# qope/SIPP

Measured on NVIDIA B200. Metric: SIPP native prove throughput (pairings aggregated per second), higher is better.
Workload: dtype u32 limbs (254-bit modular integer)

## Files before the change

### include/sipp_b200.h

```cpp
#ifndef SIPP_B200_H
#define SIPP_B200_H
#include <stddef.h>
#include <stdint.h>

#ifdef __cplusplus
extern "C" {
#endif

typedef enum {
    SIPP_OK = 0,
    SIPP_ERR_CUDA = -1,
    SIPP_ERR_ARG = -2,
    SIPP_ERR_LENGTH = -3,
    SIPP_ERR_ZERO_CHALLENGE = -4,
    SIPP_ERR_SHORT_PROOF = -5,
    SIPP_ERR_ENCODING = -6,
    SIPP_ERR_VERIFY = -7,
    SIPP_ERR_COMM = -8
} sipp_status;

typedef struct sipp_ctx sipp_ctx;

int sipp_init(int device);
int sipp_shutdown(void);
const char *sipp_last_error(void);
int sipp_device_count(void);

#define SIPP_OPT_FE_NORMALISATION 1
#define SIPP_OPT_FQ12_ORDER 2
#define SIPP_OPT_PROFILE 3
#define SIPP_OPT_PIPELINE 4
#define SIPP_OPT_WIDE_LINES_MAX 5
#define SIPP_OPT_FE_ENGINE 6
#define SIPP_OPT_WIDE_FOLD_MAX 7
#define SIPP_OPT_WIDE_ACCUM_MAX 8
#define SIPP_OPT_BATCH_KPG_MAX 9
#define SIPP_OPT_FOLD_STRAUS 10
#define SIPP_OPT_BATCH_STREAMS 11
#define SIPP_OPT_BATCH_QLINES 12
#define SIPP_OPT_VALIDATE_POINTS 13
#define SIPP_OPT_MATRIX_TAIL 14
#define SIPP_OPT_MATRIX_BLOCK_N 15
#define SIPP_OPT_MATRIX_FIRST 17
#define SIPP_OPT_MATRIX_BLOCK_R 16
int sipp_set_option(int option, int value);
int sipp_get_option(int option);

int sipp_ctx_create(const uint8_t *A, const uint8_t *B, size_t n, sipp_ctx **out);
int sipp_ctx_create_from_device(const void *dA, const void *dB, size_t n, sipp_ctx **out);
int sipp_ctx_destroy(sipp_ctx *ctx);
size_t sipp_ctx_len(const sipp_ctx *ctx);
int sipp_ctx_inner_product(sipp_ctx *ctx, uint8_t out[384]);
int sipp_ctx_cross_products(sipp_ctx *ctx, uint8_t zl[384], uint8_t zr[384]);
int sipp_ctx_fold(sipp_ctx *ctx, const uint8_t x[32], const uint8_t x_inv[32]);
int sipp_ctx_set_stages(sipp_ctx *ctx, int on);
int sipp_ctx_read(sipp_ctx *ctx, uint8_t *A_out, uint8_t *B_out);

#define SIPP_PARTIAL_BYTES 384
int sipp_ctx_partial_products(sipp_ctx *ctx, int which, void *d_out, void *stream);
int sipp_combine_partials(const void *d_partials, int count, int nprod, uint8_t *out, void *stream);

#define SIPP_COMM_ID_BYTES 128
int sipp_comm_get_unique_id(uint8_t id[SIPP_COMM_ID_BYTES]);
int sipp_comm_init(const uint8_t id[SIPP_COMM_ID_BYTES], int rank, int world);
typedef int (*sipp_allgather_fn)(void *user, const void *send, void *recv, size_t bytes);
typedef int (*sipp_broadcast_fn)(void *user, void *buf, size_t bytes, int root);
int sipp_comm_init_host(int rank, int world, sipp_allgather_fn allgather, sipp_broadcast_fn broadcast, void *user);
int sipp_comm_destroy(void);
int sipp_comm_rank(void);
int sipp_comm_world(void);
int sipp_comm_nccl_version(void);
int sipp_prove_native_sharded(const uint8_t *A_local, const uint8_t *B_local, size_t n, const uint8_t *A_full, const uint8_t *B_full,
                              uint8_t *proof);
int sipp_prove_native_sharded_device(const void *dA_local, const void *dB_local, size_t n, const uint8_t *A_full, const uint8_t *B_full,
                                     uint8_t *proof);
#define SIPP_SHARD_XS_BYTES 72
typedef struct sipp_shard_backend {
    void *user;
    int rank, world;
    size_t (*local_len)(void *user);
    int (*products)(void *user, int which);
    int (*combine)(void *user, int nprod, uint8_t *out);
    int (*broadcast)(void *user, uint8_t *xs);
    int (*fold)(void *user, const uint8_t *x, const uint8_t *x_inv);
    int (*collapse)(void *user);
} sipp_shard_backend;
int sipp_prove_native_sharded_backend(const sipp_shard_backend *backend, size_t n, const uint8_t *A_full, const uint8_t *B_full,
                                      uint8_t *proof);

int sipp_pairing(const uint8_t a[64], const uint8_t b[128], uint8_t out[384]);
int sipp_inner_product(const uint8_t *A, const uint8_t *B, size_t n, uint8_t out[384]);
int sipp_fr_inverse(const uint8_t x[32], uint8_t out[32]);
int sipp_gt_fold(const uint8_t zl[384], const uint8_t z[384], const uint8_t zr[384], const uint8_t x[32],
                 const uint8_t x_inv[32], uint8_t out[384]);

typedef struct { uint64_t state[4]; } sipp_transcript;
void sipp_transcript_new(sipp_transcript *t);
void sipp_transcript_append(sipp_transcript *t, const uint64_t *msg, size_t n);
void sipp_transcript_append_fq12(sipp_transcript *t, const uint8_t f[384]);
void sipp_transcript_append_g1(sipp_transcript *t, const uint8_t a[64]);
void sipp_transcript_append_g2(sipp_transcript *t, const uint8_t b[128]);
void sipp_transcript_get_challenge(const sipp_transcript *t, uint8_t x[32]);
void sipp_transcript_append_pairs(sipp_transcript *t, const uint8_t *A, const uint8_t *B, size_t n);
void sipp_poseidon_permute(uint64_t state[12]);
void sipp_poseidon_permute_portable(uint64_t state[12]);
int sipp_poseidon_backend(void);
double sipp_poseidon_ns_per_permutation(long count);

int sipp_prove_native(const uint8_t *A, size_t a_len, const uint8_t *B, size_t b_len, uint8_t *proof);
size_t sipp_proof_len(size_t n);
int sipp_ctx_prove(sipp_ctx *ctx, const uint8_t *A, const uint8_t *B, uint8_t *proof);
int sipp_verify_native(const uint8_t *A, size_t a_len, const uint8_t *B, size_t b_len, const uint8_t *proof, size_t proof_len,
                       uint8_t *final_A, uint8_t *final_B, uint8_t *final_Z);

size_t sipp_statement_u32_len(size_t n);
int sipp_statement_to_u32(const uint8_t *A, const uint8_t *B, size_t n, const uint8_t Z[384], const uint8_t final_A[64],
                          const uint8_t final_B[128], const uint8_t final_Z[384], uint32_t *out, size_t out_len);
int sipp_statement_from_u32(size_t n, const uint32_t *in, size_t in_len, uint8_t *A, uint8_t *B, uint8_t Z[384], uint8_t final_A[64],
                            uint8_t final_B[128], uint8_t final_Z[384]);

int sipp_prove_native_batch(const uint8_t *A, const uint8_t *B, size_t n, size_t count, uint8_t *proofs);
int sipp_verify_native_batch(const uint8_t *A, const uint8_t *B, size_t n, size_t count, const uint8_t *proofs, size_t proof_len,
                             int *results, uint8_t *final_A, uint8_t *final_B, uint8_t *final_Z);
int sipp_prove_native_batch_device(const void *dA, const void *dB, size_t n, size_t count, void *d_proofs);

int sipp_g1_generator_mul_batch(const uint8_t *scalars, size_t count, uint8_t *out);
int sipp_g1_generator_mul_batch_device(const void *d_scalars, size_t count, void *d_out);
int sipp_g2_mul_batch(const uint8_t *points, size_t point_count, const uint8_t *scalars, size_t count, uint8_t *out);
int sipp_g2_mul_batch_device(const void *d_points, size_t point_count, const void *d_scalars, size_t count, void *d_out);
int sipp_g2_sum(const uint8_t *points, size_t count, uint8_t out[128]);
int sipp_g2_sum_device(const void *d_points, size_t count, void *d_out);
int sipp_g1_neg_generator(uint8_t out[64]);

int sipp_seeded_inputs_device(uint64_t seed, size_t n, void *dA, void *dB);
int sipp_seeded_inputs(uint64_t seed, size_t n, uint8_t *A, uint8_t *B);

typedef struct {
    uint64_t launches;
    uint64_t miller_pairs;
    uint64_t miller_launches;
    double miller_ms;
    double reduce_fe_ms;
    double fold_ms;
    uint64_t fold_points;
    double transcript_ms;
    double other_ms;
} sipp_stats;
int sipp_get_stats(sipp_stats *out);
int sipp_reset_stats(void);

int sipp_test_fq_op(int op, const uint8_t *a, const uint8_t *b, uint8_t *out, size_t count);
int sipp_test_fq12_op(int op, const uint8_t *a, const uint8_t *b, uint8_t *out, size_t count);
int sipp_test_fold_plan(const uint8_t x[32], const uint8_t x_inv[32], uint32_t *out_words, size_t out_cap);
int sipp_test_poseidon_device(uint64_t *states, size_t count);
int sipp_test_transcript_round_device(uint64_t *states, const uint8_t *fq12s, int nf, size_t count, uint8_t *x_out, uint32_t *plans_out);
int sipp_test_fr_inverse_binary(const uint8_t x[32], uint8_t out[32]);
int sipp_microbench(int which, int iters, double *ops_per_s, double *ms);
long sipp_test_stage_blocks(int which, size_t n);
long sipp_test_poseidon_chain(uint64_t seed, long count);
int sipp_test_poseidon_scalar(int which, const uint64_t *in, uint64_t *out);
const void *sipp_test_poseidon_tables(void);

#ifdef __cplusplus
}
#endif
#endif
```

### sipp_b200/_lib.py

```python
import ctypes
import os

_HERE = os.path.dirname(os.path.abspath(__file__))
LIB_PATH = os.environ.get("SIPP_LIB") or os.path.join(_HERE, "libsipp_b200.so")

OK, ERR_CUDA, ERR_ARG, ERR_LENGTH, ERR_ZERO_CHALLENGE, ERR_SHORT_PROOF, ERR_ENCODING, ERR_VERIFY, ERR_COMM = 0, -1, -2, -3, -4, -5, -6, -7, -8
OPT_FE_NORMALISATION, OPT_FQ12_ORDER, OPT_PROFILE, OPT_PIPELINE, OPT_WIDE_LINES_MAX, OPT_FE_ENGINE, OPT_WIDE_FOLD_MAX, OPT_WIDE_ACCUM_MAX = 1, 2, 3, 4, 5, 6, 7, 8
OPT_BATCH_KPG_MAX, OPT_FOLD_STRAUS, OPT_BATCH_STREAMS, OPT_BATCH_QLINES, OPT_VALIDATE_POINTS, OPT_MATRIX_TAIL, OPT_MATRIX_BLOCK_N, OPT_MATRIX_BLOCK_R, OPT_MATRIX_FIRST = 9, 10, 11, 12, 13, 14, 15, 16, 17


class SippError(RuntimeError):
    def __init__(self, code, msg):
        super().__init__("libsipp_b200 error %d: %s" % (code, msg))
        self.code = code


class Stats(ctypes.Structure):
    _fields_ = [("launches", ctypes.c_uint64), ("miller_pairs", ctypes.c_uint64), ("miller_launches", ctypes.c_uint64),
                ("miller_ms", ctypes.c_double), ("reduce_fe_ms", ctypes.c_double), ("fold_ms", ctypes.c_double),
                ("fold_points", ctypes.c_uint64), ("transcript_ms", ctypes.c_double), ("other_ms", ctypes.c_double)]


class TranscriptState(ctypes.Structure):
    _fields_ = [("state", ctypes.c_uint64 * 4)]


ALLGATHER_FN = ctypes.CFUNCTYPE(ctypes.c_int, ctypes.c_void_p, ctypes.c_void_p, ctypes.c_void_p, ctypes.c_size_t)
BROADCAST_FN = ctypes.CFUNCTYPE(ctypes.c_int, ctypes.c_void_p, ctypes.c_void_p, ctypes.c_size_t, ctypes.c_int)
SHARD_XS_BYTES = 72


class ShardBackend(ctypes.Structure):
    LEN_FN = ctypes.CFUNCTYPE(ctypes.c_size_t, ctypes.c_void_p)
    PRODUCTS_FN = ctypes.CFUNCTYPE(ctypes.c_int, ctypes.c_void_p, ctypes.c_int)
    COMBINE_FN = ctypes.CFUNCTYPE(ctypes.c_int, ctypes.c_void_p, ctypes.c_int, ctypes.c_void_p)
    BROADCAST_FN = ctypes.CFUNCTYPE(ctypes.c_int, ctypes.c_void_p, ctypes.c_void_p)
    FOLD_FN = ctypes.CFUNCTYPE(ctypes.c_int, ctypes.c_void_p, ctypes.c_void_p, ctypes.c_void_p)
    COLLAPSE_FN = ctypes.CFUNCTYPE(ctypes.c_int, ctypes.c_void_p)
    _fields_ = [("user", ctypes.c_void_p), ("rank", ctypes.c_int), ("world", ctypes.c_int), ("local_len", LEN_FN), ("products", PRODUCTS_FN),
                ("combine", COMBINE_FN), ("broadcast", BROADCAST_FN), ("fold", FOLD_FN), ("collapse", COLLAPSE_FN)]


_lib = None


def load():
    global _lib
    if _lib is not None:
        return _lib
    if not os.path.exists(LIB_PATH):
        raise SippError(ERR_CUDA, "%s not built: run `python -c 'import __graft_entry__ as g; g.build()'` "
                                  "(there is no CPU fallback)" % LIB_PATH)
    lib = ctypes.CDLL(LIB_PATH)
    vp, sz, u8p, i = ctypes.c_void_p, ctypes.c_size_t, ctypes.c_char_p, ctypes.c_int
    lib.sipp_last_error.restype = ctypes.c_char_p
    lib.sipp_ctx_create.argtypes = [u8p, u8p, sz, ctypes.POINTER(vp)]
    lib.sipp_poseidon_ns_per_permutation.argtypes = [ctypes.c_long]
    lib.sipp_poseidon_ns_per_permutation.restype = ctypes.c_double
    lib.sipp_ctx_create_from_device.argtypes = [vp, vp, sz, ctypes.POINTER(vp)]
    lib.sipp_ctx_destroy.argtypes = [vp]
    lib.sipp_ctx_len.argtypes = [vp]
    lib.sipp_ctx_len.restype = sz
    lib.sipp_ctx_inner_product.argtypes = [vp, u8p]
    lib.sipp_ctx_cross_products.argtypes = [vp, u8p, u8p]
    lib.sipp_ctx_fold.argtypes = [vp, u8p, u8p]
    lib.sipp_ctx_read.argtypes = [vp, u8p, u8p]
    lib.sipp_ctx_set_stages.argtypes = [vp, ctypes.c_int]
    lib.sipp_ctx_partial_products.argtypes = [vp, i, vp, vp]
    lib.sipp_combine_partials.argtypes = [vp, i, i, u8p, vp]
    lib.sipp_pairing.argtypes = [u8p, u8p, u8p]
    lib.sipp_inner_product.argtypes = [u8p, u8p, sz, u8p]
    lib.sipp_fr_inverse.argtypes = [u8p, u8p]
    lib.sipp_gt_fold.argtypes = [u8p, u8p, u8p, u8p, u8p, u8p]
    lib.sipp_transcript_new.argtypes = [ctypes.POINTER(TranscriptState)]
    lib.sipp_transcript_new.restype = None
    lib.sipp_transcript_append.argtypes = [ctypes.POINTER(TranscriptState), ctypes.POINTER(ctypes.c_uint64), sz]
    lib.sipp_transcript_append.restype = None
    for name in ("sipp_transcript_append_fq12", "sipp_transcript_append_g1", "sipp_transcript_append_g2"):
        getattr(lib, name).argtypes = [ctypes.POINTER(TranscriptState), u8p]
        getattr(lib, name).restype = None
    lib.sipp_transcript_get_challenge.argtypes = [ctypes.POINTER(TranscriptState), u8p]
    lib.sipp_transcript_get_challenge.restype = None
    lib.sipp_transcript_append_pairs.argtypes = [ctypes.POINTER(TranscriptState), u8p, u8p, sz]
    lib.sipp_transcript_append_pairs.restype = None
    lib.sipp_poseidon_permute.argtypes = [ctypes.POINTER(ctypes.c_uint64)]
    lib.sipp_poseidon_permute.restype = None
    lib.sipp_prove_native.argtypes = [u8p, sz, u8p, sz, u8p]
    lib.sipp_proof_len.argtypes = [sz]
    lib.sipp_proof_len.restype = sz
    lib.sipp_ctx_prove.argtypes = [vp, u8p, u8p, u8p]
    lib.sipp_verify_native.argtypes = [u8p, sz, u8p, sz, u8p, sz, u8p, u8p, u8p]
    lib.sipp_seeded_inputs_device.argtypes = [ctypes.c_uint64, sz, vp, vp]
    lib.sipp_seeded_inputs.argtypes = [ctypes.c_uint64, sz, u8p, u8p]
    lib.sipp_get_stats.argtypes = [ctypes.POINTER(Stats)]
    lib.sipp_test_fq_op.argtypes = [i, u8p, u8p, u8p, sz]
    lib.sipp_test_fq12_op.argtypes = [i, u8p, u8p, u8p, sz]
    lib.sipp_prove_native_batch.argtypes = [u8p, u8p, sz, sz, u8p]
    lib.sipp_prove_native_batch_device.argtypes = [vp, vp, sz, sz, vp]
    lib.sipp_verify_native_batch.argtypes = [u8p, u8p, sz, sz, u8p, sz, ctypes.POINTER(ctypes.c_int), u8p, u8p, u8p]
    lib.sipp_test_poseidon_device.argtypes = [ctypes.POINTER(ctypes.c_uint64), sz]
    lib.sipp_test_transcript_round_device.argtypes = [ctypes.POINTER(ctypes.c_uint64), u8p, i, sz, u8p, ctypes.POINTER(ctypes.c_uint32)]
    lib.sipp_test_fold_plan.argtypes = [u8p, u8p, ctypes.POINTER(ctypes.c_uint32), sz]
    u32p = ctypes.POINTER(ctypes.c_uint32)
    lib.sipp_statement_u32_len.argtypes = [sz]
    lib.sipp_statement_u32_len.restype = sz
    lib.sipp_statement_to_u32.argtypes = [u8p, u8p, sz, u8p, u8p, u8p, u8p, u32p, sz]
    lib.sipp_statement_from_u32.argtypes = [sz, u32p, sz, u8p, u8p, u8p, u8p, u8p, u8p]
    lib.sipp_g1_generator_mul_batch.argtypes = [u8p, sz, u8p]
    lib.sipp_g1_generator_mul_batch_device.argtypes = [vp, sz, vp]
    lib.sipp_g2_mul_batch.argtypes = [u8p, sz, u8p, sz, u8p]
    lib.sipp_g2_mul_batch_device.argtypes = [vp, sz, vp, sz, vp]
    lib.sipp_g2_sum.argtypes = [u8p, sz, u8p]
    lib.sipp_g2_sum_device.argtypes = [vp, sz, vp]
    lib.sipp_g1_neg_generator.argtypes = [u8p]
    lib.sipp_comm_get_unique_id.argtypes = [u8p]
    lib.sipp_comm_init.argtypes = [u8p, i, i]
    lib.sipp_comm_init_host.argtypes = [i, i, ALLGATHER_FN, BROADCAST_FN, vp]
    lib.sipp_prove_native_sharded.argtypes = [u8p, u8p, sz, u8p, u8p, u8p]
    lib.sipp_prove_native_sharded_device.argtypes = [vp, vp, sz, u8p, u8p, u8p]
    lib.sipp_prove_native_sharded_backend.argtypes = [ctypes.POINTER(ShardBackend), sz, u8p, u8p, u8p]
    lib.sipp_microbench.argtypes = [i, i, ctypes.POINTER(ctypes.c_double), ctypes.POINTER(ctypes.c_double)]
    _lib = lib
    return lib


def check(rc):
    if rc != OK:
        raise SippError(rc, load().sipp_last_error().decode("utf-8", "replace"))
    return rc


def require_gpu(device=0):
    check(load().sipp_init(device))


_gpu_ready = False


def require_gpu_once():
    global _gpu_ready
    if not _gpu_ready:
        dev = int(os.environ.get("LOCAL_RANK", "0")) if "SIPP_DEVICE" not in os.environ else int(os.environ["SIPP_DEVICE"])
        require_gpu(dev)
        _gpu_ready = True
```

### sipp_b200/csrc/fold_plan.h

```cpp
#pragma once
#include <stdint.h>

namespace sipp {

#define SIPP_FOLD_MASK_WORDS 5

struct FoldSubScalar {
    uint64_t mag[3];
    int neg;
};
struct FoldComp {
    uint32_t plus[SIPP_FOLD_MASK_WORDS];
    uint32_t minus[SIPP_FOLD_MASK_WORDS];
    int neg;
};
struct FoldPlan {
    FoldComp g1[2];
    FoldComp g2[4];
    int g1_bits, g2_bits;
};

struct GtPlan {
    FoldComp c[8];
    int bits;
};

int fold_decompose_g1(const uint64_t k[4], FoldSubScalar out[2]);
int fold_decompose_g2(const uint64_t k[4], FoldSubScalar out[4]);
int fold_plan_build(const uint8_t x[32], const uint8_t x_inv[32], FoldPlan* plan);
int gt_plan_build(const uint8_t x[32], const uint8_t x_inv[32], GtPlan* plan);

}
```

### sipp_b200/csrc/glv.cc

```cpp
#include <string.h>

#include "glv_consts.h"
#include "glv_core.h"

namespace sipp {

static const glv::Tables HOST_TABLES = {&SIPP_GLV_G1_BASIS[0][0][0], &SIPP_GLV_G1_RECIP[0][0], SIPP_GLV_G1_RECIP_SIGN,
                                        &SIPP_GLS_G2_BASIS[0][0][0], &SIPP_GLS_G2_RECIP[0][0], SIPP_GLS_G2_RECIP_SIGN};

int fold_decompose_g2(const uint64_t k[4], FoldSubScalar out[4]) {
    return glv::decompose<4>(k, HOST_TABLES.g2_basis, HOST_TABLES.g2_recip, HOST_TABLES.g2_sign, out);
}
int fold_decompose_g1(const uint64_t k[4], FoldSubScalar out[2]) {
    return glv::decompose<2>(k, HOST_TABLES.g1_basis, HOST_TABLES.g1_recip, HOST_TABLES.g1_sign, out);
}

int fold_plan_build(const uint8_t x[32], const uint8_t x_inv[32], FoldPlan* plan) {
    uint64_t kx[4], ki[4];
    memcpy(kx, x, 32);
    memcpy(ki, x_inv, 32);
    memset(plan, 0, sizeof *plan);
    return glv::plan_build(kx, ki, HOST_TABLES, plan);
}

int gt_plan_build(const uint8_t x[32], const uint8_t x_inv[32], GtPlan* plan) {
    memset(plan, 0, sizeof *plan);
    for (int which = 0; which < 2; which++) {
        uint64_t k[4];
        memcpy(k, which ? x_inv : x, 32);
        FoldSubScalar s[4];
        if (fold_decompose_g2(k, s)) return -1;
        for (int j = 0; j < 4; j++) {
            FoldComp& c = plan->c[4 * which + j];
            const int len = glv::naf(s[j].mag, c.plus, c.minus);
            c.neg = s[j].neg;
            if (len > plan->bits) plan->bits = len;
        }
    }
    return plan->bits > 32 * SIPP_FOLD_MASK_WORDS ? -1 : 0;
}

}

extern "C" int sipp_test_fr_inverse_binary(const uint8_t x[32], uint8_t out[32]) {
    uint64_t v[4], o[4] = {0, 0, 0, 0};
    memcpy(v, x, 32);
    int rc = sipp::glv::fr_inverse_binary(v, o);
    memcpy(out, o, 32);
    return rc;
}
```

### sipp_b200/csrc/host_state.h

```cpp
#pragma once
#include <cuda_runtime.h>
#include <stddef.h>
#include <stdint.h>

#include <atomic>
#include <thread>

#include "../../include/sipp_b200.h"
#include "launch.h"

namespace sipp_host {
void pool_free(void* p);
struct MatTail {
    uint32_t* E[2] = {nullptr, nullptr};
    int cur = 0;
    size_t n = 0;
    size_t m = 1;
    bool fold_points = false;
    int folds = 0;
    void reset() {
        pool_free(E[0]);
        pool_free(E[1]);
        E[0] = E[1] = nullptr;
        n = 0;
        m = 1;
        fold_points = false;
    }
    ~MatTail() { reset(); }
};
}

struct sipp_ctx {
    uint32_t* dA = nullptr;
    uint32_t* dB = nullptr;
    size_t n = 0, cap = 0;
    bool stages = false;
    bool stale = false;
    bool pending_validation = false;
    cudaEvent_t validated = nullptr;
    sipp_host::MatTail mt;
};

namespace sipp_host {

extern int g_device;
extern int g_sm_count;
extern cudaStream_t g_stream;
#define SIPP_FIRST_STAGE_LOG2_LOOPS 18
size_t mat_first_budget(size_t n);
extern int g_opt_pipeline, g_opt_fe_norm, g_opt_fq12_order, g_opt_profile, g_opt_fold_straus, g_opt_batch_kpg_max, g_opt_batch_streams, g_opt_batch_qlines, g_opt_wide_max, g_opt_wide_fold_max, g_opt_fe_engine, g_opt_validate, g_opt_matrix_n, g_opt_matrix_first, g_opt_matrix_block_n, g_opt_matrix_block_r;
extern sipp_stats g_stats;

int fail(int code, const char* what);
int cuda_fail(cudaError_t e, const char* what);
int ensure_init();
bool is_pow2(size_t n);

void batch_release_streams();
int ctx_alloc(size_t n, sipp_ctx** out);
inline bool fq_bytes_canonical(const uint8_t* b, size_t n_fq) {
    static const uint64_t PM[4] = {0x3c208c16d87cfd47ull, 0x97816a916871ca8dull, 0xb85045b68181585dull, 0x30644e72e131a029ull};
    for (size_t i = 0; i < n_fq; i++) {
        uint64_t w[4];
        __builtin_memcpy(w, b + 32 * i, 32);
        bool less = false;
        for (int k = 3; k >= 0; k--) {
            if (w[k] != PM[k]) { less = w[k] < PM[k]; break; }
        }
        if (!less) return false;
    }
    return true;
}
cudaError_t pool_alloc(void** out, size_t bytes);
int lines_reserve(size_t bytes);
uint32_t* lines_buffer();
cudaError_t order_after(cudaStream_t later, cudaStream_t earlier);

struct AbsorbJob {
    sipp_transcript tr;
    std::thread th;
    std::atomic<bool> cancel{false};
    void start(const uint8_t* A, const uint8_t* B, size_t n) {
        sipp_transcript_new(&tr);
        th = std::thread([this, A, B, n]() {
            const size_t chunk = 512;
            for (size_t i = 0; i < n && !cancel.load(std::memory_order_relaxed); i += chunk)
                sipp_transcript_append_pairs(&tr, A + 64 * i, B + 128 * i, n - i < chunk ? n - i : chunk);
        });
    }
    double join();
    ~AbsorbJob() {
        cancel.store(true);
        if (th.joinable()) th.join();
    }
};

size_t mat_stage_first(size_t n);
int mat_diag_product(MatTail& mt, uint8_t* z);
size_t mat_stage(size_t n);
int mat_build(sipp_ctx* c, MatTail& mt, size_t nr);
int mat_build_ex(sipp_ctx* c, MatTail& mt, size_t nr, uint32_t* raw_out);
int mat_adopt(MatTail& mt, const uint32_t* gathered, int ranks, size_t nr);
int mat_products(MatTail& mt, uint8_t* zl, uint8_t* zr);
int mat_fold(sipp_ctx* c, MatTail& mt, const uint8_t x[32], const uint8_t xinv[32]);

int prove_core(sipp_ctx* c, AbsorbJob& job, uint8_t* proof);

int span_begin(int kind, cudaStream_t s);
void span_end(int idx, cudaStream_t s);
struct Span {
    int idx;
    cudaStream_t stream;
    Span(int kind, cudaStream_t s) : idx(span_begin(kind, s)), stream(s) {}
    ~Span() { span_end(idx, stream); }
};

}

#define CK(call)                                                    \
    do {                                                            \
        cudaError_t e_ = (call);                                    \
        if (e_ != cudaSuccess) return sipp_host::cuda_fail(e_, #call); \
    } while (0)
```

### sipp_b200/csrc/k_fold.cu

```cuda
#define SIPP_CURVE_FQ2_CALLS 1
#define SIPP_FQ_CALLS 1
#include "coop.cuh"
#include "device_common.cuh"
#include "fold_plan.h"
#include "fq2h.cuh"

namespace sipp {

#define SIPP_FOLD_THREADS 128

template <class F>
__device__ __forceinline__ void store_jac(uint32_t* dst, const Jac<F>& p);
template <>
__device__ __forceinline__ void store_jac<Fq2>(uint32_t* dst, const Jac<Fq2>& p) {
    store_fq2_words(dst, p.x); store_fq2_words(dst + 16, p.y); store_fq2_words(dst + 32, p.z);
}
__device__ __forceinline__ Jac<Fq2> load_jac2(const uint32_t* src) {
    Jac<Fq2> p;
    p.x = load_fq2_words(src); p.y = load_fq2_words(src + 16); p.z = load_fq2_words(src + 32);
    return p;
}
__device__ __forceinline__ void store_fq_words(uint32_t* p, const Fq& v) {
    uint4* q = reinterpret_cast<uint4*>(p);
    q[0] = make_uint4(v.l[0], v.l[1], v.l[2], v.l[3]);
    q[1] = make_uint4(v.l[4], v.l[5], v.l[6], v.l[7]);
}
__device__ __forceinline__ Fq load_fq_words(const uint32_t* p) {
    const uint4* q = reinterpret_cast<const uint4*>(p);
    uint4 a = q[0], b = q[1];
    return Fq{{a.x, a.y, a.z, a.w, b.x, b.y, b.z, b.w}};
}
template <>
__device__ __forceinline__ void store_jac<Fq>(uint32_t* dst, const Jac<Fq>& p) {
    store_fq_words(dst, p.x); store_fq_words(dst + 8, p.y); store_fq_words(dst + 16, p.z);
}
__device__ __forceinline__ Jac<Fq> load_jac1(const uint32_t* src) {
    Jac<Fq> p;
    p.x = load_fq_words(src); p.y = load_fq_words(src + 8); p.z = load_fq_words(src + 16);
    return p;
}

__device__ __forceinline__ void store_jac_h(uint32_t* dst, const Jac<Fq2H>& p) {
    const int o = h_odd() ? 8 : 0;
    store_fq_words(dst + o, p.x.v); store_fq_words(dst + 16 + o, p.y.v); store_fq_words(dst + 32 + o, p.z.v);
}
__device__ __forceinline__ Jac<Fq2H> load_jac_h(const uint32_t* src) {
    const int o = h_odd() ? 8 : 0;
    Jac<Fq2H> p;
    p.x.v = load_fq_words(src + o); p.y.v = load_fq_words(src + 16 + o); p.z.v = load_fq_words(src + 32 + o);
    return p;
}
__device__ __forceinline__ Affine<Fq2H> split_g2(const G2A& q) { return Affine<Fq2H>{h_split(q.x), h_split(q.y)}; }

__device__ __forceinline__ void pair_mul(const Fq& a_even, const Fq& b_even, const Fq& a_odd, const Fq& b_odd, Fq& r_even, Fq& r_odd) {
    const bool odd = h_odd();
    const Fq mine = fq_mul_call(h_select(odd, a_odd, a_even), h_select(odd, b_odd, b_even));
    const Fq other = h_partner(mine);
    r_even = h_select(odd, other, mine);
    r_odd = h_select(odd, mine, other);
}
__device__ __noinline__ Jac<Fq> jac_dbl_pair(const Jac<Fq>& p) {
    Fq A, B, C, S, Fv, YZ, M, unused;
    pair_mul(p.x, p.x, p.y, p.y, A, B);
    const Fq xb = fq_add(p.x, B);
    pair_mul(B, B, xb, xb, C, S);
    const Fq D = fq_dbl(fq_sub(fq_sub(S, A), C));
    const Fq E = fq_add(fq_dbl(A), A);
    pair_mul(E, E, p.y, p.z, Fv, YZ);
    Jac<Fq> r;
    r.x = fq_sub(Fv, fq_dbl(D));
    const Fq dx = fq_sub(D, r.x);
    pair_mul(E, dx, E, dx, M, unused);
    r.y = fq_sub(M, fq_dbl(fq_dbl(fq_dbl(C))));
    r.z = fq_dbl(YZ);
    return r;
}
__device__ __noinline__ Jac<Fq> jac_add_affine_pair(const Jac<Fq>& p, const G1A& q) {
    if (affine_is_identity(q)) return p;
    if (fq_is_zero(p.z)) return Jac<Fq>{q.x, q.y, fq_one()};
    Fq zz, yz, u2, s2, hh, zh, hhh, v, r2, yh, M, unused;
    pair_mul(p.z, p.z, q.y, p.z, zz, yz);
    pair_mul(q.x, zz, yz, zz, u2, s2);
    const Fq h = fq_sub(u2, p.x), rr = fq_sub(s2, p.y);
    if (fq_is_zero(h)) {
        if (fq_is_zero(rr)) return jac_dbl_pair(p);
        return jac_identity<Fq>();
    }
    pair_mul(h, h, p.z, h, hh, zh);
    pair_mul(hh, h, p.x, hh, hhh, v);
    pair_mul(rr, rr, p.y, hhh, r2, yh);
    Jac<Fq> r;
    r.x = fq_sub(fq_sub(fq_sub(r2, hhh), v), v);
    const Fq vx = fq_sub(v, r.x);
    pair_mul(rr, vx, rr, vx, M, unused);
    r.y = fq_sub(M, yh);
    r.z = zh;
    return r;
}
__device__ __forceinline__ Jac<Fq> jac_scalar_mul_naf_pair(const G1A& q, const uint32_t* plus, const uint32_t* minus, int bits) {
    Jac<Fq> acc = jac_identity<Fq>();
    for (int i = bits - 1; i >= 0; i--) {
        acc = jac_dbl_pair(acc);
        const uint32_t m = 1u << (i & 31);
        const bool dp = (plus[i >> 5] & m) != 0, dm = (minus[i >> 5] & m) != 0;
        if (dp || dm) {
            G1A t = q;
            if (dm) t.y = fq_neg(q.y);
            acc = jac_add_affine_pair(acc, t);
        }
    }
    return acc;
}

template <class F>
__device__ __forceinline__ Jac<F> fold_component(const Affine<F>& p2, const FoldComp& c, int j, int bits) {
    Affine<F> q = endo_apply(p2, j);
    if (c.neg) q.y = f_neg(q.y);
    return jac_scalar_mul_naf(q, c.plus, c.minus, bits);
}

__global__ void __launch_bounds__(SIPP_FOLD_THREADS) k_fold_split(uint32_t* __restrict__ A, uint32_t* __restrict__ B, size_t h, FoldPlan plan_arg,
                                                                 unsigned g2_blocks) {
    __shared__ FoldPlan plan;
    __shared__ __align__(16) uint32_t xch[3 * 32 * 48];
    for (int i = threadIdx.x; i < (int)(sizeof(FoldPlan) / 4); i += blockDim.x) ((uint32_t*)&plan)[i] = ((const uint32_t*)&plan_arg)[i];
    __syncthreads();
    const int warp = threadIdx.x >> 5, lane = threadIdx.x & 31;
    if (blockIdx.x < g2_blocks) {
        const int el = lane >> 1;
        size_t i = (size_t)blockIdx.x * 16 + el;
        const bool valid = i < h;
        if (!valid) i = h - 1;
        G2A q = endo_apply(load_g2(B, i + h), warp);
        if (plan.g2[warp].neg) q.y = f_neg(q.y);
        Jac<Fq2H> acc = jac_scalar_mul_naf(split_g2(q), plan.g2[warp].plus, plan.g2[warp].minus, plan.g2_bits);
        if (warp > 0) store_jac_h(xch + ((warp - 1) * 16 + el) * 48, acc);
        __syncthreads();
        if (warp == 0) {
#pragma unroll 1
            for (int j = 0; j < 3; j++) acc = jac_add(acc, load_jac_h(xch + (j * 16 + el) * 48));
            const Affine<Fq2H> r = jac_to_affine(jac_add_affine(acc, split_g2(load_g2(B, i))));
            if (valid) {
                const int o = h_odd() ? 8 : 0;
                store_fq_words(B + 32 * i + o, r.x.v);
                store_fq_words(B + 32 * i + 16 + o, r.y.v);
            }
        }
    } else {
        const int comp = warp & 1, half = warp >> 1, el = lane >> 1;
        size_t i = (size_t)(blockIdx.x - g2_blocks) * 32 + half * 16 + el;
        const bool valid = i < h;
        if (!valid) i = h - 1;
        G1A q = endo_apply(load_g1(A, i + h), comp);
        if (plan.g1[comp].neg) q.y = fq_neg(q.y);
        Jac<Fq> acc = jac_scalar_mul_naf_pair(q, plan.g1[comp].plus, plan.g1[comp].minus, plan.g1_bits);
        if (comp == 1 && !h_odd()) store_jac(xch + (half * 16 + el) * 24, acc);
        __syncthreads();
        if (comp == 0 && !h_odd()) {
            acc = jac_add(acc, load_jac1(xch + (half * 16 + el) * 24));
            G1A r = jac_to_affine(jac_add_affine(acc, load_g1(A, i)));
            if (valid) store_g1(A, i, r);
        }
    }
}


__global__ void __launch_bounds__(SIPP_FOLD_THREADS) k_fold_batch(uint32_t* __restrict__ A, uint32_t* __restrict__ B, size_t h, size_t stride, size_t count,
                                                                 const FoldPlan* __restrict__ plans, unsigned g2_blocks) {
    __shared__ __align__(16) uint32_t xch[3 * 16 * 48];
    const int warp = threadIdx.x >> 5, lane = threadIdx.x & 31, el = lane >> 1;
    const size_t total = count * h;
    if (blockIdx.x < g2_blocks) {
        size_t e = (size_t)blockIdx.x * 16 + el;
        const bool valid = e < total;
        if (!valid) e = total - 1;
        const size_t inst = e / h, i = inst * stride + e % h;
        const FoldPlan* pl = plans + inst;
        G2A q = endo_apply(load_g2(B, i + h), warp);
        if (pl->g2[warp].neg) q.y = f_neg(q.y);
        Jac<Fq2H> acc = jac_scalar_mul_naf(split_g2(q), pl->g2[warp].plus, pl->g2[warp].minus, pl->g2_bits);
        if (warp > 0) store_jac_h(xch + ((warp - 1) * 16 + el) * 48, acc);
        __syncthreads();
        if (warp == 0) {
#pragma unroll 1
            for (int j = 0; j < 3; j++) acc = jac_add(acc, load_jac_h(xch + (j * 16 + el) * 48));
            const Affine<Fq2H> r = jac_to_affine(jac_add_affine(acc, split_g2(load_g2(B, i))));
            if (valid) {
                const int o = h_odd() ? 8 : 0;
                store_fq_words(B + 32 * i + o, r.x.v);
                store_fq_words(B + 32 * i + 16 + o, r.y.v);
            }
        }
    } else {
        const int comp = warp & 1, half = warp >> 1;
        size_t e = (size_t)(blockIdx.x - g2_blocks) * 32 + half * 16 + el;
        const bool valid = e < total;
        if (!valid) e = total - 1;
        const size_t inst = e / h, i = inst * stride + e % h;
        const FoldPlan* pl = plans + inst;
        G1A q = endo_apply(load_g1(A, i + h), comp);
        if (pl->g1[comp].neg) q.y = fq_neg(q.y);
        Jac<Fq> acc = jac_scalar_mul_naf_pair(q, pl->g1[comp].plus, pl->g1[comp].minus, pl->g1_bits);
        if (comp == 1 && !h_odd()) store_jac(xch + (half * 16 + el) * 24, acc);
        __syncthreads();
        if (comp == 0 && !h_odd()) {
            acc = jac_add(acc, load_jac1(xch + (half * 16 + el) * 24));
            G1A r = jac_to_affine(jac_add_affine(acc, load_g1(A, i)));
            if (valid) store_g1(A, i, r);
        }
    }
}

#define SIPP_STRAUS_THREADS 64

__global__ void __launch_bounds__(SIPP_STRAUS_THREADS) k_fold_straus(uint32_t* __restrict__ A, uint32_t* __restrict__ B, size_t h, size_t stride, size_t count,
                                                                   const FoldPlan* __restrict__ plans, unsigned g2_blocks) {
    const size_t total = count * h;
    const bool is_g2 = blockIdx.x < g2_blocks;
    size_t e = (size_t)(is_g2 ? blockIdx.x : blockIdx.x - g2_blocks) * SIPP_STRAUS_THREADS + threadIdx.x;
    if (e >= total) return;
    const size_t inst = e / h, i = inst * stride + e % h;
    const FoldPlan* pl = plans + inst;
    if (is_g2) {
        G2A tbl[4];
        const G2A p2 = load_g2(B, i + h);
#pragma unroll 1
        for (int c = 0; c < 4; c++) {
            tbl[c] = endo_apply(p2, c);
            if (pl->g2[c].neg) tbl[c].y = f_neg(tbl[c].y);
        }
        Jac<Fq2> acc = straus_naf<Fq2, 4>(tbl, pl->g2, pl->g2_bits);
        store_g2(B, i, jac_to_affine(jac_add_affine(acc, load_g2(B, i))));
    } else {
        G1A tbl[2];
        const G1A p2 = load_g1(A, i + h);
#pragma unroll 1
        for (int c = 0; c < 2; c++) {
            tbl[c] = endo_apply(p2, c);
            if (pl->g1[c].neg) tbl[c].y = f_neg(tbl[c].y);
        }
        Jac<Fq> acc = straus_naf<Fq, 2>(tbl, pl->g1, pl->g1_bits);
        store_g1(A, i, jac_to_affine(jac_add_affine(acc, load_g1(A, i))));
    }
}

__device__ __forceinline__ Jac<Fq2> psi_jac(const Jac<Fq2>& p, int j) {
    Jac<Fq2> r;
    r.x = f_mul((j & 1) ? fq2_conj(p.x) : p.x, frob_gamma(j, 2));
    r.y = f_mul((j & 1) ? fq2_conj(p.y) : p.y, frob_gamma(j, 3));
    r.z = (j & 1) ? fq2_conj(p.z) : p.z;
    return r;
}
__device__ bool jac_equal(const Jac<Fq2>& p, const Jac<Fq2>& q) {
    const bool pz = f_is_zero(p.z), qz = f_is_zero(q.z);
    if (pz || qz) return pz && qz;
    const Fq2 z1 = f_sqr(p.z), z2 = f_sqr(q.z);
    if (!fq2_eq(f_mul(p.x, z2), f_mul(q.x, z1))) return false;
    return fq2_eq(f_mul(p.y, f_mul(z2, q.z)), f_mul(q.y, f_mul(z1, p.z)));
}
__global__ void __launch_bounds__(64) k_validate_points(const uint32_t* __restrict__ dA, const uint32_t* __restrict__ dB, size_t n, int* __restrict__ flags) {
    const size_t t = (size_t)blockIdx.x * blockDim.x + threadIdx.x;
    if (t >= 2 * n) return;
    if (t < n) {
        const G1A p{load_fq_words(dA + 16 * t), load_fq_words(dA + 16 * t + 8)};
        if (affine_is_identity(p)) return;
        const Fq three = fq_to_mont(Fq{{3, 0, 0, 0, 0, 0, 0, 0}});
        if (!f_is_zero(f_sub(f_sqr(p.y), f_add(f_mul(f_sqr(p.x), p.x), three)))) atomicOr(flags, 2);
        return;
    }
    const size_t i = t - n;
    const G2A q{load_fq2_words(dB + 32 * i), load_fq2_words(dB + 32 * i + 16)};
    if (affine_is_identity(q)) return;
    if (!fq2_eq(f_sqr(q.y), f_add(f_mul(f_sqr(q.x), q.x), fq2_b_twist()))) { atomicOr(flags, 2); return; }
    const unsigned long long xb = SIPP_BN_X;
    const uint32_t k[8] = {(uint32_t)xb, (uint32_t)(xb >> 32), 0, 0, 0, 0, 0, 0};
    const Jac<Fq2> xq = jac_scalar_mul(q, k);
    Jac<Fq2> lhs = jac_add_affine(xq, q);
    lhs = jac_add(lhs, psi_jac(xq, 1));
    lhs = jac_add(lhs, psi_jac(xq, 2));
    const Jac<Fq2> rhs = psi_jac(jac_dbl(xq), 3);
    if (!jac_equal(lhs, rhs)) atomicOr(flags, 4);
}
int launch_validate_points(const uint32_t* dA, const uint32_t* dB, size_t n, int* flags, cudaStream_t s) {
    k_validate_points<<<(unsigned)((2 * n + 63) / 64), 64, 0, s>>>(dA, dB, n, flags);
    return (int)cudaGetLastError();
}

int launch_fold(uint32_t* A, uint32_t* B, size_t h, const FoldPlan& plan, cudaStream_t s) {
    unsigned g2_blocks = (unsigned)((h + 15) / 16), g1_blocks = (unsigned)((h + 31) / 32);
    k_fold_split<<<g2_blocks + g1_blocks, SIPP_FOLD_THREADS, 0, s>>>(A, B, h, plan, g2_blocks);
    return (int)cudaGetLastError();
}
int launch_fold_batch(uint32_t* A, uint32_t* B, size_t h, size_t stride, size_t count, const FoldPlan* plans, cudaStream_t s) {
    size_t total = count * h;
    unsigned g2_blocks = (unsigned)((total + 15) / 16), g1_blocks = (unsigned)((total + 31) / 32);
    k_fold_batch<<<g2_blocks + g1_blocks, SIPP_FOLD_THREADS, 0, s>>>(A, B, h, stride, count, plans, g2_blocks);
    return (int)cudaGetLastError();
}
int launch_fold_straus(uint32_t* A, uint32_t* B, size_t h, size_t stride, size_t count, const FoldPlan* plans, cudaStream_t s) {
    size_t total = count * h;
    unsigned blocks = (unsigned)((total + SIPP_STRAUS_THREADS - 1) / SIPP_STRAUS_THREADS);
    k_fold_straus<<<2 * blocks, SIPP_STRAUS_THREADS, 0, s>>>(A, B, h, stride, count, plans, blocks);
    return (int)cudaGetLastError();
}

}
```

### sipp_b200/csrc/k_wide.cu

```cuda
#include "engine.cuh"
#include "device_common.cuh"

namespace sipp {

#define SIPP_WIDE_THREADS 128
#define SIPP_WIDE_GROUPS (SIPP_WIDE_THREADS / SIPP_LP_LANES)
#define SIPP_LINE_WORDS 80

static __device__ const LpIns d_lp_code[SIPP_LP_LEVELS * SIPP_LP_LANES] = SIPP_LP_CODE_INIT;
static __constant__ unsigned char c_lp_types[SIPP_LP_LEVELS] = SIPP_LP_TYPES_INIT;

struct DevMachine {
    uint32_t* slots;
    uint32_t* out;
    int lane;
    bool store, ident;
    __device__ __forceinline__ void run(int first, int n) {
#pragma unroll 1
        for (int L = first; L < first + n; L++) {
            const uint4 w = __ldg(reinterpret_cast<const uint4*>(d_lp_code) + L * SIPP_LP_LANES + lane);
            const LpIns ins{w.x, w.y, w.z, w.w};
            const Fq r = lp_eval(c_lp_types[L], ins, slots);
            __syncwarp();
            lp_store(slots, lp_dst(ins), r);
            __syncwarp();
        }
    }
    __device__ __forceinline__ void emit(int step) {
        if (lane < 10 && store) {
            Fq v = lp_load(slots, SIPP_LP_SLOT_OUT0 + lane);
            if (ident) v = (lane == 0) ? fq_one() : fq_zero();
            uint4* o = reinterpret_cast<uint4*>(out + (size_t)step * SIPP_LINE_WORDS + lane * 8);
            o[0] = make_uint4(v.l[0], v.l[1], v.l[2], v.l[3]);
            o[1] = make_uint4(v.l[4], v.l[5], v.l[6], v.l[7]);
        }
    }
};

__global__ void __launch_bounds__(SIPP_WIDE_THREADS) k_lines_wide(const uint32_t* __restrict__ A, const uint32_t* __restrict__ B, MillerJob job, int nprod,
                                                                 size_t c0, size_t mc, uint32_t* __restrict__ lines) {
    __shared__ __align__(16) uint32_t smem[SIPP_WIDE_GROUPS * SIPP_LP_SLOTS * 8];
    __shared__ int ident_flag[SIPP_WIDE_GROUPS];
    const int group = threadIdx.x / SIPP_LP_LANES, lane = threadIdx.x % SIPP_LP_LANES;
    const size_t total = mc * (size_t)nprod;
    size_t t = (size_t)blockIdx.x * SIPP_WIDE_GROUPS + group;
    const bool valid = t < total;
    if (!valid) t = total - 1;
    const int prod = (int)(t / mc);
    const size_t j = c0 + (t - (size_t)prod * mc);
    uint32_t* slots = smem + group * (SIPP_LP_SLOTS * 8);
    if (lane == 0) {
        const G1A p = load_g1(A, job.a_off[prod] + j);
        const G2A q = load_g2(B, job.b_off[prod] + j);
        ident_flag[group] = (affine_is_identity(p) || affine_is_identity(q)) ? 1 : 0;
        lp_fill_fixed(slots, p.x, p.y, q.x, q.y);
    }
    __syncwarp();
    DevMachine mach;
    mach.slots = slots;
    mach.out = lines + t * (size_t)(SIPP_LINES_PER_PAIR * SIPP_LINE_WORDS);
    mach.lane = lane;
    mach.store = valid;
    mach.ident = ident_flag[group] != 0;
    lp_miller(mach);
}

__global__ void __launch_bounds__(SIPP_WIDE_THREADS) k_lines_wide_batch(const uint32_t* __restrict__ A, const uint32_t* __restrict__ B, BatchJob job, size_t p0,
                                                                       size_t np, uint32_t* __restrict__ lines) {
    __shared__ __align__(16) uint32_t smem[SIPP_WIDE_GROUPS * SIPP_LP_SLOTS * 8];
    __shared__ int ident_flag[SIPP_WIDE_GROUPS];
    const int group = threadIdx.x / SIPP_LP_LANES, lane = threadIdx.x % SIPP_LP_LANES;
    const size_t total = np * job.h;
    size_t t = (size_t)blockIdx.x * SIPP_WIDE_GROUPS + group;
    const bool valid = t < total;
    if (!valid) t = total - 1;
    const size_t P = p0 + t / job.h, i = t % job.h;
    const size_t inst = P / (size_t)job.nprod;
    const int y = (int)(P % (size_t)job.nprod);
    const size_t base = inst * job.stride + i;
    uint32_t* slots = smem + group * (SIPP_LP_SLOTS * 8);
    if (lane == 0) {
        const G1A p = load_g1(A, base + job.a_off[y]);
        const G2A q = load_g2(B, base + job.b_off[y]);
        ident_flag[group] = (affine_is_identity(p) || affine_is_identity(q)) ? 1 : 0;
        lp_fill_fixed(slots, p.x, p.y, q.x, q.y);
    }
    __syncwarp();
    DevMachine mach;
    mach.slots = slots;
    mach.out = lines + t * (size_t)(SIPP_LINES_PER_PAIR * SIPP_LINE_WORDS);
    mach.lane = lane;
    mach.store = valid;
    mach.ident = ident_flag[group] != 0;
    lp_miller(mach);
}

int launch_lines_wide_batch(const uint32_t* A, const uint32_t* B, const BatchJob& job, size_t p0, size_t np, uint32_t* lines, cudaStream_t s) {
    const size_t groups = np * job.h;
    k_lines_wide_batch<<<(unsigned)((groups + SIPP_WIDE_GROUPS - 1) / SIPP_WIDE_GROUPS), SIPP_WIDE_THREADS, 0, s>>>(A, B, job, p0, np, lines);
    return (int)cudaGetLastError();
}

int launch_lines_wide(const uint32_t* A, const uint32_t* B, const MillerJob& job, int nprod, size_t c0, size_t mc, uint32_t* lines, cudaStream_t s) {
    const size_t groups = mc * (size_t)nprod;
    k_lines_wide<<<(unsigned)((groups + SIPP_WIDE_GROUPS - 1) / SIPP_WIDE_GROUPS), SIPP_WIDE_THREADS, 0, s>>>(A, B, job, nprod, c0, mc, lines);
    return (int)cudaGetLastError();
}

}

namespace sipp {

__device__ __forceinline__ void store_words(uint32_t* dst, const Fq& v) {
#pragma unroll
    for (int i = 0; i < 8; i++) dst[i] = v.l[i];
}
__device__ __forceinline__ Fq load_words(const uint32_t* src) {
    Fq v;
#pragma unroll
    for (int i = 0; i < 8; i++) v.l[i] = src[i];
    return v;
}

__global__ void __launch_bounds__(SIPP_WIDE_THREADS) k_fold_wide(uint32_t* __restrict__ A, uint32_t* __restrict__ B, size_t h, FoldPlan plan_arg, unsigned g2_blocks) {
    __shared__ __align__(16) uint32_t smem[SIPP_WIDE_GROUPS * SIPP_LP_SLOTS * 8];
    __shared__ FoldPlan plan;
    __shared__ __align__(16) uint32_t xch[SIPP_WIDE_GROUPS * 48];
    for (int i = threadIdx.x; i < (int)(sizeof(FoldPlan) / 4); i += blockDim.x) ((uint32_t*)&plan)[i] = ((const uint32_t*)&plan_arg)[i];
    __syncthreads();
    const int warp = threadIdx.x >> 5, group = threadIdx.x / SIPP_LP_LANES, lane = threadIdx.x % SIPP_LP_LANES, gi = group & 1;
    uint32_t* slots = smem + group * (SIPP_LP_SLOTS * 8);
    DevMachine mach;
    mach.slots = slots; mach.out = nullptr; mach.lane = lane; mach.store = false; mach.ident = false;
    if (blockIdx.x < g2_blocks) {
        const int comp = warp;
        size_t e = (size_t)blockIdx.x * 2 + gi;
        const bool valid = e < h;
        if (!valid) e = h - 1;
        const FoldDigits d = fold_digits(plan.g2[comp], plan.g2_bits);
        bool ident = false;
        if (lane == 0) {
            G2A q = load_g2(B, e + h);
            ident = affine_is_identity(q);
            q = endo_apply(q, comp);
            if ((plan.g2[comp].neg != 0) != d.flip) q.y = fq2_neg(q.y);
            lp_fill_fixed(slots, fq_zero(), fq_zero(), q.x, q.y);
        }
        __syncwarp();
        if (d.top >= 0) {
            mach.run(SIPP_LP_SETUP_FIRST, SIPP_LP_SETUP_LEVELS);
            lp_scalar_mul(mach, true, d.plus, d.minus, d.top);
        }
        if (lane == 0) {
            Jac<Fq2> r = jac_identity<Fq2>();
            if (!ident && d.top >= 0) {
                const Fq2 X{lp_load(slots, SIPP_LP_SLOT_X0), lp_load(slots, SIPP_LP_SLOT_X1)}, Y{lp_load(slots, SIPP_LP_SLOT_Y0), lp_load(slots, SIPP_LP_SLOT_Y1)};
                const Fq2 Z = fq2_mul_xi(Fq2{lp_load(slots, SIPP_LP_SLOT_ZH0), lp_load(slots, SIPP_LP_SLOT_ZH1)});
                r.x = fq2_mul(X, Z);
                r.y = fq2_mul(Y, fq2_sqr(Z));
                r.z = Z;
            }
            uint32_t* o = xch + group * 48;
            store_words(o, r.x.c0); store_words(o + 8, r.x.c1); store_words(o + 16, r.y.c0); store_words(o + 24, r.y.c1);
            store_words(o + 32, r.z.c0); store_words(o + 40, r.z.c1);
        }
        __syncthreads();
        if (warp == 0 && lane == 0) {
            Jac<Fq2> acc;
            for (int j = 0; j < 4; j++) {
                const uint32_t* o = xch + ((j * 2 + gi) * 48);
                Jac<Fq2> t;
                t.x = Fq2{load_words(o), load_words(o + 8)}; t.y = Fq2{load_words(o + 16), load_words(o + 24)}; t.z = Fq2{load_words(o + 32), load_words(o + 40)};
                acc = j ? jac_add(acc, t) : t;
            }
            const G2A r = jac_to_affine(jac_add_affine(acc, load_g2(B, e)));
            if (valid) store_g2(B, e, r);
        }
    } else {
        const int comp = warp & 1, pair = warp >> 1;
        size_t e = (size_t)(blockIdx.x - g2_blocks) * 4 + pair * 2 + gi;
        const bool valid = e < h;
        if (!valid) e = h - 1;
        const FoldDigits d = fold_digits(plan.g1[comp], plan.g1_bits);
        bool ident = false;
        if (lane == 0) {
            G1A q = load_g1(A, e + h);
            ident = affine_is_identity(q);
            q = endo_apply(q, comp);
            if ((plan.g1[comp].neg != 0) != d.flip) q.y = fq_neg(q.y);
            lp_store(slots, SIPP_LP_SLOT_ZERO, fq_zero());
            lp_store(slots, SIPP_LP_SLOT_QX0, q.x); lp_store(slots, SIPP_LP_SLOT_QY0, q.y);
            lp_store(slots, SIPP_LP_SLOT_X1, q.x); lp_store(slots, SIPP_LP_SLOT_Y1, q.y); lp_store(slots, SIPP_LP_SLOT_Z1, fq_one());
        }
        __syncwarp();
        if (d.top >= 0) lp_scalar_mul(mach, false, d.plus, d.minus, d.top);
        if (lane == 0) {
            Jac<Fq> r = jac_identity<Fq>();
            if (!ident && d.top >= 0) {
                const Fq X = lp_load(slots, SIPP_LP_SLOT_X1), Y = lp_load(slots, SIPP_LP_SLOT_Y1), Z = lp_load(slots, SIPP_LP_SLOT_Z1);
                r.x = fq_mul(X, Z);
                r.y = fq_mul(Y, fq_sqr(Z));
                r.z = Z;
            }
            uint32_t* o = xch + group * 48;
            store_words(o, r.x); store_words(o + 8, r.y); store_words(o + 16, r.z);
        }
        __syncthreads();
        if (comp == 0 && lane == 0) {
            Jac<Fq> acc, t;
            const uint32_t* o0 = xch + group * 48;
            const uint32_t* o1 = xch + (group + 2) * 48;
            acc.x = load_words(o0); acc.y = load_words(o0 + 8); acc.z = load_words(o0 + 16);
            t.x = load_words(o1); t.y = load_words(o1 + 8); t.z = load_words(o1 + 16);
            acc = jac_add(acc, t);
            const G1A r = jac_to_affine(jac_add_affine(acc, load_g1(A, e)));
            if (valid) store_g1(A, e, r);
        }
    }
}

__global__ void __launch_bounds__(SIPP_WIDE_THREADS) k_fold_wide_batch(uint32_t* __restrict__ A, uint32_t* __restrict__ B, size_t h, size_t stride, size_t count,
                                                                      const FoldPlan* __restrict__ plans, unsigned g2_blocks) {
    __shared__ __align__(16) uint32_t smem[SIPP_WIDE_GROUPS * SIPP_LP_SLOTS * 8];
    __shared__ __align__(16) uint32_t xch[SIPP_WIDE_GROUPS * 48];
    const size_t total = count * h;
    const int epw = h >= 2 ? 2 : 1;
    const int warp = threadIdx.x >> 5, group = threadIdx.x / SIPP_LP_LANES, lane = threadIdx.x % SIPP_LP_LANES, gi = group & 1;
    uint32_t* slots = smem + group * (SIPP_LP_SLOTS * 8);
    DevMachine mach;
    mach.slots = slots; mach.out = nullptr; mach.lane = lane; mach.store = false; mach.ident = false;
    if (blockIdx.x < g2_blocks) {
        const int comp = warp;
        size_t E = (size_t)blockIdx.x * epw + (gi % epw);
        const bool valid = E < total && gi < epw;
        if (E >= total) E = total - 1;
        const size_t inst = E / h, e = inst * stride + E % h;
        const FoldPlan& plan = plans[inst];
        const FoldDigits d = fold_digits(plan.g2[comp], plan.g2_bits);
        bool ident = false;
        if (lane == 0) {
            G2A q = load_g2(B, e + h);
            ident = affine_is_identity(q);
            q = endo_apply(q, comp);
            if ((plan.g2[comp].neg != 0) != d.flip) q.y = fq2_neg(q.y);
            lp_fill_fixed(slots, fq_zero(), fq_zero(), q.x, q.y);
        }
        __syncwarp();
        if (d.top >= 0) {
            mach.run(SIPP_LP_SETUP_FIRST, SIPP_LP_SETUP_LEVELS);
            lp_scalar_mul(mach, true, d.plus, d.minus, d.top);
        }
        if (lane == 0) {
            Jac<Fq2> r = jac_identity<Fq2>();
            if (!ident && d.top >= 0) {
                const Fq2 X{lp_load(slots, SIPP_LP_SLOT_X0), lp_load(slots, SIPP_LP_SLOT_X1)}, Y{lp_load(slots, SIPP_LP_SLOT_Y0), lp_load(slots, SIPP_LP_SLOT_Y1)};
                const Fq2 Z = fq2_mul_xi(Fq2{lp_load(slots, SIPP_LP_SLOT_ZH0), lp_load(slots, SIPP_LP_SLOT_ZH1)});
                r.x = fq2_mul(X, Z);
                r.y = fq2_mul(Y, fq2_sqr(Z));
                r.z = Z;
            }
            uint32_t* o = xch + group * 48;
            store_words(o, r.x.c0); store_words(o + 8, r.x.c1); store_words(o + 16, r.y.c0); store_words(o + 24, r.y.c1);
            store_words(o + 32, r.z.c0); store_words(o + 40, r.z.c1);
        }
        __syncthreads();
        if (warp == 0 && lane == 0) {
            Jac<Fq2> acc;
            for (int j = 0; j < 4; j++) {
                const uint32_t* o = xch + ((j * 2 + gi) * 48);
                Jac<Fq2> t;
                t.x = Fq2{load_words(o), load_words(o + 8)}; t.y = Fq2{load_words(o + 16), load_words(o + 24)}; t.z = Fq2{load_words(o + 32), load_words(o + 40)};
                acc = j ? jac_add(acc, t) : t;
            }
            const G2A r = jac_to_affine(jac_add_affine(acc, load_g2(B, e)));
            if (valid) store_g2(B, e, r);
        }
    } else {
        const int comp = warp & 1, pair = warp >> 1;
        size_t E = (size_t)(blockIdx.x - g2_blocks) * (2 * epw) + pair * epw + (gi % epw);
        const bool valid = E < total && gi < epw;
        if (E >= total) E = total - 1;
        const size_t inst = E / h, e = inst * stride + E % h;
        const FoldPlan& plan = plans[inst];
        const FoldDigits d = fold_digits(plan.g1[comp], plan.g1_bits);
        bool ident = false;
        if (lane == 0) {
            G1A q = load_g1(A, e + h);
            ident = affine_is_identity(q);
            q = endo_apply(q, comp);
            if ((plan.g1[comp].neg != 0) != d.flip) q.y = fq_neg(q.y);
            lp_store(slots, SIPP_LP_SLOT_ZERO, fq_zero());
            lp_store(slots, SIPP_LP_SLOT_QX0, q.x); lp_store(slots, SIPP_LP_SLOT_QY0, q.y);
            lp_store(slots, SIPP_LP_SLOT_X1, q.x); lp_store(slots, SIPP_LP_SLOT_Y1, q.y); lp_store(slots, SIPP_LP_SLOT_Z1, fq_one());
        }
        __syncwarp();
        if (d.top >= 0) lp_scalar_mul(mach, false, d.plus, d.minus, d.top);
        if (lane == 0) {
            Jac<Fq> r = jac_identity<Fq>();
            if (!ident && d.top >= 0) {
                const Fq X = lp_load(slots, SIPP_LP_SLOT_X1), Y = lp_load(slots, SIPP_LP_SLOT_Y1), Z = lp_load(slots, SIPP_LP_SLOT_Z1);
                r.x = fq_mul(X, Z);
                r.y = fq_mul(Y, fq_sqr(Z));
                r.z = Z;
            }
            uint32_t* o = xch + group * 48;
            store_words(o, r.x); store_words(o + 8, r.y); store_words(o + 16, r.z);
        }
        __syncthreads();
        if (comp == 0 && lane == 0) {
            Jac<Fq> acc, t;
            const uint32_t* o0 = xch + group * 48;
            const uint32_t* o1 = xch + (group + 2) * 48;
            acc.x = load_words(o0); acc.y = load_words(o0 + 8); acc.z = load_words(o0 + 16);
            t.x = load_words(o1); t.y = load_words(o1 + 8); t.z = load_words(o1 + 16);
            acc = jac_add(acc, t);
            const G1A r = jac_to_affine(jac_add_affine(acc, load_g1(A, e)));
            if (valid) store_g1(A, e, r);
        }
    }
}


int launch_fold_wide_batch(uint32_t* A, uint32_t* B, size_t h, size_t stride, size_t count, const FoldPlan* plans, cudaStream_t s) {
    const size_t total = count * h, epw = h >= 2 ? 2 : 1;
    const unsigned g2_blocks = (unsigned)((total + epw - 1) / epw), g1_blocks = (unsigned)((total + 2 * epw - 1) / (2 * epw));
    k_fold_wide_batch<<<g2_blocks + g1_blocks, SIPP_WIDE_THREADS, 0, s>>>(A, B, h, stride, count, plans, g2_blocks);
    return (int)cudaGetLastError();
}
int launch_fold_wide(uint32_t* A, uint32_t* B, size_t h, const FoldPlan& plan, cudaStream_t s) {
    const unsigned g2_blocks = (unsigned)((h + 1) / 2), g1_blocks = (unsigned)((h + 3) / 4);
    k_fold_wide<<<g2_blocks + g1_blocks, SIPP_WIDE_THREADS, 0, s>>>(A, B, h, plan, g2_blocks);
    return (int)cudaGetLastError();
}

}
```

### sipp_b200/csrc/launch.h

```cpp
#pragma once
#include <cuda_runtime.h>
#include <stddef.h>
#include <stdint.h>

#include "fold_plan.h"

namespace sipp {

struct MillerJob {
    size_t a_off[2];
    size_t b_off[2];
    size_t m;
};
struct BatchJob {
    size_t stride;
    size_t a_off[2];
    size_t b_off[2];
    size_t h;
    int nprod;
};
struct Scalar256 {
    uint32_t w[8];
};

#define SIPP_MILLER_BLOCK 64

int launch_codec_decode(const uint32_t* in, uint32_t* out, size_t n_fq, int* flags, cudaStream_t s);
int launch_codec_encode(const uint32_t* in, uint32_t* out, size_t n_fq, cudaStream_t s);
int launch_miller_block(const uint32_t* A, const uint32_t* B, const MillerJob& job, int nprod, uint32_t* partials, cudaStream_t s);
int launch_reduce_fe(const uint32_t* partials, int count, int nprod, uint32_t* out, int final_exp, int ark_norm, cudaStream_t s);
int launch_gt_fold(const uint32_t* in, const Scalar256& x, const Scalar256& xinv, uint32_t* out, cudaStream_t s);
int launch_gt_fold_eng(const uint32_t* in, const Scalar256& x, const Scalar256& xinv, uint32_t* out, cudaStream_t s);
int launch_gt_fold_rounds(const uint32_t* elems, const uint32_t* scalars, int rounds, uint32_t* partials, cudaStream_t s);
int launch_fold(uint32_t* A, uint32_t* B, size_t h, const FoldPlan& plan, cudaStream_t s);
int launch_fold_wide(uint32_t* A, uint32_t* B, size_t h, const FoldPlan& plan, cudaStream_t s);
int launch_validate_points(const uint32_t* dA, const uint32_t* dB, size_t n, int* flags, cudaStream_t s);
int launch_test_fq_op(int op, const uint32_t* a, const uint32_t* b, uint32_t* out, size_t count, cudaStream_t s);
int launch_test_fq12_op(int op, const uint32_t* a, const uint32_t* b, uint32_t* out, size_t count, cudaStream_t s);
int launch_microbench(int which, int blocks, int threads, void* out, int iters, uint32_t seed, double* ops_per_thread, cudaStream_t s);

int launch_lines(const uint32_t* A, const uint32_t* B, const MillerJob& job, int nprod, size_t c0, size_t mc, uint32_t* lines, cudaStream_t s);
int launch_lines_wide(const uint32_t* A, const uint32_t* B, const MillerJob& job, int nprod, size_t c0, size_t mc, uint32_t* lines, cudaStream_t s);
int accum_blocks(size_t m_chunk, int kpg);
int launch_accum(const uint32_t* lines, size_t m_chunk, int nprod, int kpg, uint32_t* partials, int block_offset, cudaStream_t s);
int launch_reduce_fe_coop(const uint32_t* partials, int count, int nprod, uint32_t* out, int final_exp, int ark_norm, cudaStream_t s);
int launch_reduce_fe_eng(const uint32_t* partials, int count, int nprod, uint32_t* out, int final_exp, int ark_norm, cudaStream_t s);
int accum_eng_blocks(size_t m_chunk, int kpg);
int launch_accum_eng(const uint32_t* lines, size_t m_chunk, int nprod, int kpg, uint32_t* partials, int block_offset, cudaStream_t s);
int launch_accum_eng_each(const uint32_t* lines, size_t m, uint32_t* out, cudaStream_t s);
int launch_test_coop_op(int op, const uint32_t* a, const uint32_t* b, uint32_t* out, size_t count, cudaStream_t s);
size_t lines_bytes_per_pair();

int launch_mat_gather(const uint32_t* A, const uint32_t* B, size_t nr, size_t m, uint32_t* Aexp, uint32_t* Bexp, cudaStream_t s);
int launch_mat_fe(const uint32_t* miller, size_t count, uint32_t* E, int ark_norm, cudaStream_t s);
int launch_mat_diag(const uint32_t* E, size_t n, int main_diagonal, uint32_t* partials, cudaStream_t s);
int launch_mat_fold(const uint32_t* E, size_t n, uint32_t* Eout, const GtPlan& plan, cudaStream_t s);

int launch_lines_batch(const uint32_t* A, const uint32_t* B, const BatchJob& job, size_t p0, size_t np, uint32_t* lines, cudaStream_t s);
int launch_accum_batch(const uint32_t* lines, size_t pairs, int kpg, uint32_t* partials, size_t group_offset, cudaStream_t s);
int launch_fe_batch(const uint32_t* partials, size_t nproducts, int gpp, int nprod, uint32_t* out, size_t out_stride, int slot0, int slot1, int ark_norm,
                    cudaStream_t s);
int launch_lines_wide_batch(const uint32_t* A, const uint32_t* B, const BatchJob& job, size_t p0, size_t np, uint32_t* lines, cudaStream_t s);
int launch_qlines_batch(const uint32_t* B, size_t npoints, uint32_t* qlines, cudaStream_t s);
int launch_eval_lines_batch(const uint32_t* A, const uint32_t* B, const BatchJob& job, size_t p0, size_t np, const uint32_t* qlines, uint32_t* lines,
                            cudaStream_t s);
size_t qlines_bytes_per_point();
int launch_eval_lines_mat(const uint32_t* A, const uint32_t* B, size_t nr, size_t m, const uint32_t* qlines, uint32_t* lines, cudaStream_t s);
int launch_fe_batch_eng(const uint32_t* partials, size_t nproducts, int gpp, int nprod, uint32_t* out, size_t out_stride, int slot0, int slot1, int ark_norm,
                        cudaStream_t s);
int launch_fold_batch(uint32_t* A, uint32_t* B, size_t h, size_t stride, size_t count, const FoldPlan* plans, cudaStream_t s);
int launch_fold_wide_batch(uint32_t* A, uint32_t* B, size_t h, size_t stride, size_t count, const FoldPlan* plans, cudaStream_t s);
int launch_fold_straus(uint32_t* A, uint32_t* B, size_t h, size_t stride, size_t count, const FoldPlan* plans, cudaStream_t s);
int launch_tr_absorb_pairs(const uint32_t* bytesA, const uint32_t* bytesB, size_t n, size_t count, uint64_t* states, cudaStream_t s);
int launch_tr_round(uint64_t* states, const uint32_t* proofs, size_t np, int slot_z, int slot_l, int slot_r, int order, size_t count, FoldPlan* plans,
                    uint64_t* challenges, int* flags, cudaStream_t s);
int launch_test_poseidon(uint64_t* states, size_t count, cudaStream_t s);
int launch_gt_fold_batch(const uint32_t* proofs, size_t stride, int slot_l, int slot_r, const uint64_t* challenges, uint32_t* z, size_t count,
                         cudaStream_t s);

size_t window_table_bytes(int group);
int launch_window_table(int group, const uint32_t* base, uint32_t* table, cudaStream_t s);
int launch_fixed_base_mul(int group, const uint32_t* table, const uint32_t* scalars, size_t count, uint32_t* out, cudaStream_t s);
int launch_g2_mul_var(const uint32_t* points, const uint32_t* scalars, size_t count, uint32_t* out, cudaStream_t s);
int g2_sum_blocks(size_t count, int sm_count);
int launch_g2_sum(const uint32_t* points, size_t count, uint32_t* partials, int blocks, uint32_t* out, cudaStream_t s);
int launch_seeded_scalars(uint64_t seed, size_t n, uint32_t* sa, uint32_t* sb, cudaStream_t s);
int launch_generators(uint32_t* gens, cudaStream_t s);

}
```

### sipp_b200/csrc/sipp_b200.cu

```cuda
#include <cuda_runtime.h>
#include <stdio.h>
#include <string.h>

#include <chrono>
#include <string>
#include <thread>
#include <vector>

#include "glv_core.h"
#include "host_state.h"

using namespace sipp;

namespace sipp_host {

thread_local std::string g_err;
int g_device = -1;
cudaStream_t g_stream = nullptr;
int g_opt_fe_norm = 0, g_opt_fq12_order = 0, g_opt_profile = 0, g_opt_pipeline = 1;
int g_opt_fe_engine = 1;
int g_opt_wide_fold_max = 256;
int g_opt_wide_accum_max = 1536;
int g_opt_wide_max = 8192;
int g_sm_count = 148;
int g_opt_fold_straus = 1;
int g_opt_batch_streams = 0;
int g_opt_batch_qlines = 1;
int g_opt_batch_kpg_max = 32;
int g_opt_matrix_n = 32;
int g_opt_matrix_first = 1;
int g_opt_matrix_block_n = 256, g_opt_matrix_block_r = 8;
int g_opt_validate = 1;

struct TimedSpan {
    cudaEvent_t a, b;
    int kind;
};
std::vector<TimedSpan> g_spans;
sipp_stats g_stats;

int fail(int code, const char* what) {
    g_err = what;
    return code;
}
int cuda_fail(cudaError_t e, const char* what) {
    g_err = std::string(what) + ": " + cudaGetErrorString(e);
    return SIPP_ERR_CUDA;
}
int ensure_init() {
    if (g_device >= 0) return SIPP_OK;
    return sipp_init(0);
}

int span_begin(int kind, cudaStream_t s) {
    if (!g_opt_profile) return -1;
    TimedSpan t;
    t.kind = kind;
    cudaEventCreate(&t.a);
    cudaEventCreate(&t.b);
    cudaEventRecord(t.a, s);
    g_spans.push_back(t);
    return (int)g_spans.size() - 1;
}
void span_end(int idx, cudaStream_t s) {
    if (idx >= 0) cudaEventRecord(g_spans[idx].b, s);
}

void collect_spans() {
    for (auto& t : g_spans) {
        cudaEventSynchronize(t.b);
        float ms = 0;
        cudaEventElapsedTime(&ms, t.a, t.b);
        if (t.kind == 0) g_stats.miller_ms += ms;
        else if (t.kind == 1) g_stats.reduce_fe_ms += ms;
        else if (t.kind == 2) g_stats.fold_ms += ms;
        else g_stats.other_ms += ms;
        cudaEventDestroy(t.a);
        cudaEventDestroy(t.b);
    }
    g_spans.clear();
}

double AbsorbJob::join() {
    if (!th.joinable()) return 0.0;
    auto t0 = std::chrono::steady_clock::now();
    th.join();
    return std::chrono::duration<double, std::milli>(std::chrono::steady_clock::now() - t0).count();
}

size_t log2_exact(size_t n) {
    size_t r = 0;
    while (n > 1) { n >>= 1; r++; }
    return r;
}
bool is_pow2(size_t n) { return n && !(n & (n - 1)); }

Scalar256 scalar_from_bytes(const uint8_t* b) {
    Scalar256 s;
    memcpy(s.w, b, 32);
    return s;
}

struct PoolBlock {
    void* ptr;
    size_t size;
    bool used;
};
std::vector<PoolBlock> g_pool;
cudaError_t pool_alloc(void** out, size_t bytes) {
    if (bytes == 0) bytes = 16;
    int best = -1;
    for (size_t i = 0; i < g_pool.size(); i++) {
        const PoolBlock& b = g_pool[i];
        if (!b.used && b.size >= bytes && b.size <= 2 * bytes && (best < 0 || b.size < g_pool[best].size)) best = (int)i;
    }
    if (best >= 0) {
        g_pool[best].used = true;
        *out = g_pool[best].ptr;
        return cudaSuccess;
    }
    void* p = nullptr;
    cudaError_t e = cudaMalloc(&p, bytes);
    if (e != cudaSuccess) return e;
    g_pool.push_back({p, bytes, true});
    *out = p;
    return cudaSuccess;
}
void pool_free(void* p) {
    if (!p) return;
    for (auto& b : g_pool)
        if (b.ptr == p) { b.used = false; return; }
    cudaFree(p);
}
void pool_release_all() {
    for (auto& b : g_pool) cudaFree(b.ptr);
    g_pool.clear();
}

struct Scratch {
    uint32_t* partials = nullptr;
    size_t partial_blocks = 0;
    uint32_t* out = nullptr;
    uint8_t* h_out = nullptr;
    int* flag = nullptr;
    int* vflag = nullptr;
    uint32_t* lines = nullptr;
    size_t lines_bytes = 0;
} g_scr;

int scratch_reserve(size_t blocks) {
    if (!g_scr.out) {
        CK(cudaMalloc(&g_scr.out, 4 * 96 * sizeof(uint32_t)));
        CK(cudaMallocHost(&g_scr.h_out, 4 * 384));
        CK(cudaMalloc(&g_scr.flag, sizeof(int)));
        CK(cudaMalloc(&g_scr.vflag, sizeof(int)));
    }
    if (blocks > g_scr.partial_blocks) {
        if (g_scr.partials) CK(cudaFree(g_scr.partials));
        size_t cap = blocks < 1024 ? 1024 : blocks;
        CK(cudaMalloc(&g_scr.partials, cap * 2 * 96 * sizeof(uint32_t)));
        g_scr.partial_blocks = cap;
    }
    return SIPP_OK;
}

int lines_reserve(size_t bytes) {
    if (bytes > g_scr.lines_bytes) {
        if (g_scr.lines) CK(cudaFree(g_scr.lines));
        g_scr.lines = nullptr;
        g_scr.lines_bytes = 0;
        CK(cudaMalloc(&g_scr.lines, bytes));
        g_scr.lines_bytes = bytes;
    }
    return SIPP_OK;
}

uint32_t* lines_buffer() { return g_scr.lines; }

cudaError_t order_after(cudaStream_t later, cudaStream_t earlier) {
    cudaEvent_t ev;
    cudaError_t e = cudaEventCreateWithFlags(&ev, cudaEventDisableTiming);
    if (e != cudaSuccess) return e;
    e = cudaEventRecord(ev, earlier);
    if (e == cudaSuccess) e = cudaStreamWaitEvent(later, ev, 0);
    cudaEventDestroy(ev);
    return e;
}


}
using namespace sipp_host;

namespace {

int launch_decode(const uint32_t* d_bytes, uint32_t* d_out, size_t n_fq, cudaStream_t s, bool check) {
    if (check) CK(cudaMemsetAsync(g_scr.flag, 0, sizeof(int), s));
    Span sp(3, s);
    int e = launch_codec_decode(d_bytes, d_out, n_fq, check ? g_scr.flag : nullptr, s);
    if (e) return cuda_fail((cudaError_t)e, "k_codec_decode");
    g_stats.launches++;
    return SIPP_OK;
}

int launch_miller(const sipp_ctx* c, int nprod, const MillerJob& job, uint32_t* d_partials, size_t* blocks_out, cudaStream_t s) {
    size_t blocks = (job.m + SIPP_MILLER_BLOCK - 1) / SIPP_MILLER_BLOCK;
    {
        Span sp(0, s);
        int e = launch_miller_block(c->dA, c->dB, job, nprod, d_partials, s);
        if (e) return cuda_fail((cudaError_t)e, "k_miller_block");
    }
    g_stats.launches++;
    g_stats.miller_launches++;
    g_stats.miller_pairs += job.m * (size_t)nprod;
    *blocks_out = blocks;
    return SIPP_OK;
}

int launch_reduce(const uint32_t* d_partials, int count, int nprod, uint32_t* d_out, bool final_exp, cudaStream_t s) {
    Span sp(1, s);
    int e = !g_opt_pipeline ? launch_reduce_fe(d_partials, count, nprod, d_out, final_exp ? 1 : 0, g_opt_fe_norm, s)
            : g_opt_fe_engine ? launch_reduce_fe_eng(d_partials, count, nprod, d_out, final_exp ? 1 : 0, g_opt_fe_norm, s)
                              : launch_reduce_fe_coop(d_partials, count, nprod, d_out, final_exp ? 1 : 0, g_opt_fe_norm, s);
    if (e) return cuda_fail((cudaError_t)e, "k_reduce_fe");
    g_stats.launches++;
    return SIPP_OK;
}

int ctx_products_to_device(sipp_ctx* c, int which, size_t* blocks_out, int* nprod_out, cudaStream_t s) {
    MillerJob job;
    int nprod;
    if (which == 0) {
        nprod = 1;
        job.a_off[0] = 0; job.b_off[0] = 0; job.a_off[1] = 0; job.b_off[1] = 0;
        job.m = c->n;
    } else {
        if (c->n < 2) return fail(SIPP_ERR_ARG, "cross products need n >= 2");
        size_t h = c->n / 2;
        nprod = 2;
        job.a_off[0] = h; job.b_off[0] = 0;
        job.a_off[1] = 0; job.b_off[1] = h;
        job.m = h;
    }
    *nprod_out = nprod;
    if (!g_opt_pipeline) {
        size_t blocks = (job.m + SIPP_MILLER_BLOCK - 1) / SIPP_MILLER_BLOCK;
        int rc = scratch_reserve(blocks);
        if (rc) return rc;
        return launch_miller(c, nprod, job, g_scr.partials, blocks_out, s);
    }
    const size_t per_pair = lines_bytes_per_pair();
    const size_t cap_bytes = (size_t)6 << 30;
    size_t mc = job.m;
    if (mc * (size_t)nprod * per_pair > cap_bytes) mc = cap_bytes / ((size_t)nprod * per_pair);
    const bool eng = mc * (size_t)nprod <= (size_t)g_opt_wide_accum_max;
    const size_t groups_target = eng ? (size_t)g_sm_count * 8 : (size_t)g_sm_count * 2 * 20;
    int kpg = (int)(((eng ? mc * (size_t)nprod : mc) + groups_target - 1) / groups_target);
    if (kpg < 1) kpg = 1;
    auto blocks_of = [&](size_t cur) { return (size_t)(eng ? accum_eng_blocks(cur, kpg) : accum_blocks(cur, kpg)); };
    size_t total_blocks = 0;
    for (size_t c0 = 0; c0 < job.m; c0 += mc) {
        size_t cur = job.m - c0 < mc ? job.m - c0 : mc;
        total_blocks += blocks_of(cur);
    }
    int rc = scratch_reserve(total_blocks);
    if (rc) return rc;
    rc = lines_reserve(mc * (size_t)nprod * per_pair);
    if (rc) return rc;
    size_t block_off = 0;
    for (size_t c0 = 0; c0 < job.m; c0 += mc) {
        size_t cur = job.m - c0 < mc ? job.m - c0 : mc;
        Span sp(0, s);
        const bool wide = cur * (size_t)nprod <= (size_t)g_opt_wide_max;
        int e = wide ? launch_lines_wide(c->dA, c->dB, job, nprod, c0, cur, g_scr.lines, s) : launch_lines(c->dA, c->dB, job, nprod, c0, cur, g_scr.lines, s);
        if (e) return cuda_fail((cudaError_t)e, "k_lines");
        e = eng ? launch_accum_eng(g_scr.lines, cur, nprod, kpg, g_scr.partials, (int)block_off, s)
                : launch_accum(g_scr.lines, cur, nprod, kpg, g_scr.partials, (int)block_off, s);
        if (e) return cuda_fail((cudaError_t)e, "k_accum");
        block_off += blocks_of(cur);
        g_stats.launches += 2;
        g_stats.miller_launches++;
    }
    g_stats.miller_pairs += job.m * (size_t)nprod;
    *blocks_out = total_blocks;
    return SIPP_OK;
}

int ctx_products(sipp_ctx* c, int which, uint8_t* out0, uint8_t* out1) {
    size_t blocks;
    int nprod;
    int rc = ctx_products_to_device(c, which, &blocks, &nprod, g_stream);
    if (rc) return rc;
    rc = launch_reduce(g_scr.partials, (int)blocks, nprod, g_scr.out, true, g_stream);
    if (rc) return rc;
    CK(cudaMemcpyAsync(g_scr.h_out, g_scr.out, (size_t)nprod * 384, cudaMemcpyDeviceToHost, g_stream));
    CK(cudaStreamSynchronize(g_stream));
    memcpy(out0, g_scr.h_out, 384);
    if (nprod == 2) memcpy(out1, g_scr.h_out + 384, 384);
    return SIPP_OK;
}

}

namespace sipp_host {
cudaStream_t g_fold_stream = nullptr;
FoldPlan* g_fold_plan_dev = nullptr;
int g_live_ctx = 0;

size_t mat_stage(size_t n) {
    if (!g_opt_pipeline || !g_opt_fe_engine || n < 2) return 0;
    if (n <= (size_t)g_opt_matrix_n) return n;
    if (g_opt_matrix_n < 2 || n > (size_t)g_opt_matrix_block_n) return 0;
    size_t nr = n / 16;
    if (nr > (size_t)g_opt_matrix_block_r) nr = (size_t)g_opt_matrix_block_r;
    while (nr >= 4 && n / nr < 2) nr >>= 1;
    return nr >= 4 ? nr : 0;
}

size_t mat_first_budget(size_t n) {
    if (g_opt_matrix_first >= 10) return (size_t)1 << g_opt_matrix_first;
    const size_t by_n = n <= 256 ? 16 * n : n < 4096 ? n * (n / 128) : 32 * n, cap = (size_t)1 << SIPP_FIRST_STAGE_LOG2_LOOPS;
    return by_n < cap ? by_n : cap;
}
size_t mat_stage_first(size_t n) {
    if (!g_opt_matrix_first || !g_opt_pipeline || !g_opt_fe_engine || n < 2 || g_opt_matrix_n < 2) return 0;
    if (n <= (size_t)g_opt_matrix_n) return n;
    size_t nr = n / 32;
    if (nr < 8) nr = 8;
    if (nr > 32) nr = 32;
    while (nr > 1 && nr * n > mat_first_budget(n)) nr >>= 1;
    while (nr >= 4 && n / nr < 2) nr >>= 1;
    return nr >= 4 ? nr : 0;
}

int mat_build(sipp_ctx* c, MatTail& mt, size_t nr) { return mat_build_ex(c, mt, nr, nullptr); }

int mat_build_ex(sipp_ctx* c, MatTail& mt, size_t nr, uint32_t* raw_out) {
    const size_t n = c->n, m = n / nr, P = nr * nr, pairs = P * m;
    const bool big = m > 1 && pairs > 8192;
    int kpg = 1;
    if (big) {
        const size_t by_block = (m + 19) / 20, by_fill = (pairs + 11839) / 11840;
        kpg = (int)(by_block < by_fill ? by_block : by_fill);
        if (kpg < 1) kpg = 1;
    }
    const size_t blocks = big ? (size_t)accum_blocks(m, kpg) : (size_t)accum_eng_blocks(m, 1);
    uint32_t *aexp = nullptr, *bexp = nullptr, *mil = nullptr, *ql = nullptr, *prod = nullptr;
    int rc = scratch_reserve(m == 1 ? nr : (blocks * P + 1) / 2);
    if (!rc) rc = lines_reserve(pairs * lines_bytes_per_pair());
    if (rc) return rc;
    cudaError_t e = cudaSuccess;
    if (!raw_out) {
        e = pool_alloc((void**)&mt.E[0], P * 384);
        if (e == cudaSuccess) e = pool_alloc((void**)&mt.E[1], (P / 4) * 384);
    }
    if (e == cudaSuccess && !big) e = pool_alloc((void**)&aexp, pairs * 64);
    if (e == cudaSuccess && !big) e = pool_alloc((void**)&bexp, pairs * 128);
    if (e == cudaSuccess && big) e = pool_alloc((void**)&ql, n * qlines_bytes_per_point());
    if (e == cudaSuccess && m == 1 && !raw_out) e = pool_alloc((void**)&mil, P * 384);
    if (m == 1 && raw_out) mil = raw_out;
    int le = 0;
    if (e == cudaSuccess) {
        {
            Span sp(0, g_stream);
            if (big) {
                le = launch_qlines_batch(c->dB, n, ql, g_stream);
                if (!le) le = launch_eval_lines_mat(c->dA, c->dB, nr, m, ql, g_scr.lines, g_stream);
                if (!le) le = launch_accum(g_scr.lines, m, (int)P, kpg, g_scr.partials, 0, g_stream);
            } else {
                MillerJob job;
                job.a_off[0] = job.b_off[0] = job.a_off[1] = job.b_off[1] = 0;
                job.m = pairs;
                le = launch_mat_gather(c->dA, c->dB, nr, m, aexp, bexp, g_stream);
                if (!le)
                    le = pairs <= (size_t)g_opt_wide_max ? launch_lines_wide(aexp, bexp, job, 1, 0, pairs, g_scr.lines, g_stream)
                                                         : launch_lines(aexp, bexp, job, 1, 0, pairs, g_scr.lines, g_stream);
                if (!le) le = m == 1 ? launch_accum_eng_each(g_scr.lines, P, mil, g_stream) : launch_accum_eng(g_scr.lines, m, (int)P, 1, g_scr.partials, 0, g_stream);
            }
        }
        if (!le && raw_out) {
            Span sp(1, g_stream);
            if (m > 1) le = launch_reduce_fe_eng(g_scr.partials, (int)blocks, (int)P, raw_out, 0, g_opt_fe_norm, g_stream);
        } else if (!le) {
            Span sp(1, g_stream);
            const uint32_t* src = m == 1 ? mil : g_scr.partials;
            if (m > 1 && blocks > 1) {
                if (pool_alloc((void**)&prod, P * 384) != cudaSuccess) le = (int)cudaErrorMemoryAllocation;
                if (!le) le = launch_reduce_fe_eng(g_scr.partials, (int)blocks, (int)P, prod, 0, g_opt_fe_norm, g_stream);
                src = prod;
                g_stats.launches++;
            }
            if (!le) le = launch_mat_fe(src, P, mt.E[0], g_opt_fe_norm, g_stream);
        }
        g_stats.launches += 4;
        g_stats.miller_launches++;
        g_stats.miller_pairs += pairs;
    }
    pool_free(aexp);
    pool_free(bexp);
    if (mil != raw_out) pool_free(mil);
    pool_free(ql);
    pool_free(prod);
    if (e != cudaSuccess) return cuda_fail(e, "cudaMalloc(pairing matrix)");
    if (le) return cuda_fail((cudaError_t)le, "pairing matrix");
    if (raw_out) return SIPP_OK;
    mt.n = nr;
    mt.m = m;
    mt.fold_points = m > 1;
    mt.cur = 0;
    mt.folds = 0;
    return SIPP_OK;
}

int mat_adopt(MatTail& mt, const uint32_t* gathered, int ranks, size_t nr) {
    const size_t P = nr * nr;
    int rc = scratch_reserve(nr);
    if (rc) return rc;
    cudaError_t e = pool_alloc((void**)&mt.E[0], P * 384);
    if (e == cudaSuccess) e = pool_alloc((void**)&mt.E[1], (P / 4) * 384);
    if (e != cudaSuccess) return cuda_fail(e, "cudaMalloc(pairing matrix)");
    {
        Span sp(1, g_stream);
        int le = launch_reduce_fe_eng(gathered, ranks, (int)P, mt.E[0], 3, g_opt_fe_norm, g_stream);
        if (le) return cuda_fail((cudaError_t)le, "pairing matrix (gathered)");
    }
    g_stats.launches++;
    mt.n = nr;
    mt.m = 2;
    mt.fold_points = true;
    mt.cur = 0;
    mt.folds = 0;
    return SIPP_OK;
}

int mat_diag_product(MatTail& mt, uint8_t* z) {
    {
        Span sp(1, g_stream);
        int le = launch_mat_diag(mt.E[mt.cur], mt.n, 1, g_scr.partials, g_stream);
        if (!le) le = launch_reduce_fe_eng(g_scr.partials, (int)mt.n, 1, g_scr.out, 2, g_opt_fe_norm, g_stream);
        if (le) return cuda_fail((cudaError_t)le, "matrix diagonal");
    }
    g_stats.launches += 2;
    CK(cudaMemcpyAsync(g_scr.h_out, g_scr.out, 384, cudaMemcpyDeviceToHost, g_stream));
    CK(cudaStreamSynchronize(g_stream));
    memcpy(z, g_scr.h_out, 384);
    return SIPP_OK;
}

int mat_products(MatTail& mt, uint8_t* zl, uint8_t* zr) {
    const size_t h = mt.n / 2;
    {
        Span sp(1, g_stream);
        int le = launch_mat_diag(mt.E[mt.cur], mt.n, 0, g_scr.partials, g_stream);
        if (!le) le = launch_reduce_fe_eng(g_scr.partials, (int)h, 2, g_scr.out, 2, g_opt_fe_norm, g_stream);
        if (le) return cuda_fail((cudaError_t)le, "matrix products");
    }
    g_stats.launches += 2;
    CK(cudaMemcpyAsync(g_scr.h_out, g_scr.out, 2 * 384, cudaMemcpyDeviceToHost, g_stream));
    CK(cudaStreamSynchronize(g_stream));
    memcpy(zl, g_scr.h_out, 384);
    memcpy(zr, g_scr.h_out + 384, 384);
    return SIPP_OK;
}

int mat_fold(sipp_ctx* c, MatTail& mt, const uint8_t x[32], const uint8_t xinv[32]) {
    if (mt.n > 2) {
        GtPlan plan;
        if (gt_plan_build(x, xinv, &plan)) return fail(SIPP_ERR_ENCODING, "fold scalar out of range (must be < r)");
        Span sp(2, g_stream);
        int le = launch_mat_fold(mt.E[mt.cur], mt.n, mt.E[mt.cur ^ 1], plan, g_stream);
        if (le) return cuda_fail((cudaError_t)le, "k_mat_fold");
        g_stats.launches++;
        mt.cur ^= 1;
    }
    const size_t h = c->n / 2;
    if (mt.fold_points) {
        FoldPlan fp;
        if (fold_plan_build(x, xinv, &fp)) return fail(SIPP_ERR_ENCODING, "fold scalar out of range (must be < r)");
        if (!g_fold_stream) CK(cudaStreamCreateWithFlags(&g_fold_stream, cudaStreamNonBlocking));
        if (mt.folds++ == 0) CK(order_after(g_fold_stream, g_stream));
        Span sp(2, g_fold_stream);
        int le = h <= (size_t)g_opt_wide_fold_max ? launch_fold_wide(c->dA, c->dB, h, fp, g_fold_stream) : launch_fold(c->dA, c->dB, h, fp, g_fold_stream);
        if (le) return cuda_fail((cudaError_t)le, "k_fold (look-ahead stage)");
        g_stats.launches++;
    }
    if (!mt.fold_points) c->stale = true;
    g_stats.fold_points += h;
    c->n = h;
    mt.n /= 2;
    if (mt.n == 1) {
        if (mt.fold_points) CK(order_after(g_stream, g_fold_stream));
        mt.reset();
    }
    return SIPP_OK;
}

int ctx_alloc(size_t n, sipp_ctx** out) {
    sipp_ctx* c = new sipp_ctx();
    g_live_ctx++;
    c->n = c->cap = n;
    cudaError_t e = pool_alloc((void**)&c->dA, n * 16 * sizeof(uint32_t));
    if (e == cudaSuccess) e = pool_alloc((void**)&c->dB, n * 32 * sizeof(uint32_t));
    if (e != cudaSuccess) {
        pool_free(c->dA);
        delete c;
        g_live_ctx--;
        return cuda_fail(e, "cudaMalloc(ctx)");
    }
    *out = c;
    return SIPP_OK;
}
}

extern "C" {

const char* sipp_last_error(void) { return g_err.c_str(); }

int sipp_device_count(void) {
    int n = 0;
    if (cudaGetDeviceCount(&n) != cudaSuccess) return 0;
    return n;
}

int sipp_init(int device) {
    int n = sipp_device_count();
    if (n <= 0) return fail(SIPP_ERR_CUDA, "no CUDA device: libsipp_b200 has no CPU fallback");
    if (device < 0 || device >= n) return fail(SIPP_ERR_ARG, "device index out of range");
    if (g_device >= 0 && g_device != device) {
        if (g_live_ctx > 0) return fail(SIPP_ERR_ARG, "sipp_init: contexts of the current device are still alive (destroy them before switching devices)");
        CK(cudaSetDevice(g_device));
        sipp_shutdown();
    }
    CK(cudaSetDevice(device));
    if (!g_stream) CK(cudaStreamCreateWithFlags(&g_stream, cudaStreamNonBlocking));
    cudaDeviceProp prop;
    CK(cudaGetDeviceProperties(&prop, device));
    g_sm_count = prop.multiProcessorCount;
    g_device = device;
    return SIPP_OK;
}

int sipp_shutdown(void) {
    if (g_device < 0) return SIPP_OK;
    collect_spans();
    sipp_comm_destroy();
    if (g_scr.partials) cudaFree(g_scr.partials);
    if (g_scr.out) cudaFree(g_scr.out);
    if (g_scr.h_out) cudaFreeHost(g_scr.h_out);
    if (g_scr.flag) cudaFree(g_scr.flag);
    if (g_scr.vflag) cudaFree(g_scr.vflag);
    if (g_scr.lines) cudaFree(g_scr.lines);
    g_scr = Scratch();
    pool_release_all();
    batch_release_streams();
    if (g_fold_plan_dev) cudaFree(g_fold_plan_dev);
    g_fold_plan_dev = nullptr;
    if (g_stream) cudaStreamDestroy(g_stream);
    g_stream = nullptr;
    if (g_fold_stream) cudaStreamDestroy(g_fold_stream);
    g_fold_stream = nullptr;
    g_device = -1;
    return SIPP_OK;
}

int sipp_set_option(int option, int value) {
    switch (option) {
        case SIPP_OPT_FE_NORMALISATION: g_opt_fe_norm = value ? 1 : 0; return SIPP_OK;
        case SIPP_OPT_FQ12_ORDER: g_opt_fq12_order = value ? 1 : 0; return SIPP_OK;
        case SIPP_OPT_PROFILE: g_opt_profile = value ? 1 : 0; return SIPP_OK;
        case SIPP_OPT_PIPELINE: g_opt_pipeline = value ? 1 : 0; return SIPP_OK;
        case SIPP_OPT_WIDE_LINES_MAX: g_opt_wide_max = value < 0 ? 0 : value; return SIPP_OK;
        case SIPP_OPT_FE_ENGINE: g_opt_fe_engine = value ? 1 : 0; return SIPP_OK;
        case SIPP_OPT_WIDE_FOLD_MAX: g_opt_wide_fold_max = value < 0 ? 0 : value; return SIPP_OK;
        case SIPP_OPT_WIDE_ACCUM_MAX: g_opt_wide_accum_max = value < 0 ? 0 : value; return SIPP_OK;
        case SIPP_OPT_BATCH_KPG_MAX: g_opt_batch_kpg_max = value < 1 ? 1 : value; return SIPP_OK;
        case SIPP_OPT_FOLD_STRAUS: g_opt_fold_straus = value ? 1 : 0; return SIPP_OK;
        case SIPP_OPT_BATCH_STREAMS: g_opt_batch_streams = value < 0 ? 0 : value; return SIPP_OK;
        case SIPP_OPT_BATCH_QLINES: g_opt_batch_qlines = value ? 1 : 0; return SIPP_OK;
        case SIPP_OPT_VALIDATE_POINTS: g_opt_validate = value ? 1 : 0; return SIPP_OK;
        case SIPP_OPT_MATRIX_TAIL:
            if (value < 0 || value > 64 || (value & (value - 1))) return fail(SIPP_ERR_ARG, "SIPP_OPT_MATRIX_TAIL: 0 or a power of two <= 64");
            g_opt_matrix_n = value;
            return SIPP_OK;
        case SIPP_OPT_MATRIX_FIRST: g_opt_matrix_first = (value >= 10 && value <= 24) ? value : (value ? 1 : 0); return SIPP_OK;
        case SIPP_OPT_MATRIX_BLOCK_N: g_opt_matrix_block_n = value < 0 ? 0 : (value > 4096 ? 4096 : value); return SIPP_OK;
        case SIPP_OPT_MATRIX_BLOCK_R:
            if (value < 4 || value > 32 || (value & (value - 1))) return fail(SIPP_ERR_ARG, "SIPP_OPT_MATRIX_BLOCK_R: 4, 8, 16 or 32");
            g_opt_matrix_block_r = value;
            return SIPP_OK;
        default: return fail(SIPP_ERR_ARG, "unknown option");
    }
}
long sipp_test_stage_blocks(int which, size_t n) { return (long)(which == 0 ? mat_stage_first(n) : mat_stage(n)); }
int sipp_get_option(int option) {
    switch (option) {
        case SIPP_OPT_FE_NORMALISATION: return g_opt_fe_norm;
        case SIPP_OPT_FQ12_ORDER: return g_opt_fq12_order;
        case SIPP_OPT_PROFILE: return g_opt_profile;
        case SIPP_OPT_PIPELINE: return g_opt_pipeline;
        case SIPP_OPT_WIDE_LINES_MAX: return g_opt_wide_max;
        case SIPP_OPT_FE_ENGINE: return g_opt_fe_engine;
        case SIPP_OPT_WIDE_FOLD_MAX: return g_opt_wide_fold_max;
        case SIPP_OPT_WIDE_ACCUM_MAX: return g_opt_wide_accum_max;
        case SIPP_OPT_BATCH_KPG_MAX: return g_opt_batch_kpg_max;
        case SIPP_OPT_FOLD_STRAUS: return g_opt_fold_straus;
        case SIPP_OPT_BATCH_STREAMS: return g_opt_batch_streams;
        case SIPP_OPT_BATCH_QLINES: return g_opt_batch_qlines;
        case SIPP_OPT_VALIDATE_POINTS: return g_opt_validate;
        case SIPP_OPT_MATRIX_TAIL: return g_opt_matrix_n;
        case SIPP_OPT_MATRIX_FIRST: return g_opt_matrix_first;
        case SIPP_OPT_MATRIX_BLOCK_N: return g_opt_matrix_block_n;
        case SIPP_OPT_MATRIX_BLOCK_R: return g_opt_matrix_block_r;
        default: return -1;
    }
}

int sipp_get_stats(sipp_stats* out) {
    if (!out) return fail(SIPP_ERR_ARG, "null stats");
    if (g_device >= 0) collect_spans();
    *out = g_stats;
    return SIPP_OK;
}
int sipp_reset_stats(void) {
    if (g_device >= 0) collect_spans();
    memset(&g_stats, 0, sizeof g_stats);
    return SIPP_OK;
}

static int ctx_create_from_device_ex(const void* dA, const void* dB, size_t n, sipp_ctx** out, bool defer) {
    int rc = ensure_init();
    if (rc) return rc;
    if (!dA || !dB || !out || n == 0) return fail(SIPP_ERR_ARG, "sipp_ctx_create: null pointer or n == 0");
    rc = scratch_reserve(1);
    if (rc) return rc;
    sipp_ctx* c;
    rc = ctx_alloc(n, &c);
    if (rc) return rc;
    launch_decode((const uint32_t*)dA, c->dA, n * 2, g_stream, true);
    launch_codec_decode((const uint32_t*)dB, c->dB, n * 4, g_scr.flag, g_stream);
    g_stats.launches++;
    cudaError_t e = cudaSuccess;
    if (g_opt_validate) {
        if (defer) {
            if (!g_fold_stream) e = cudaStreamCreateWithFlags(&g_fold_stream, cudaStreamNonBlocking);
            if (e == cudaSuccess) e = order_after(g_fold_stream, g_stream);
            if (e == cudaSuccess) e = cudaMemsetAsync(g_scr.vflag, 0, sizeof(int), g_fold_stream);
            if (e == cudaSuccess) {
                Span sp(3, g_fold_stream);
                launch_validate_points(c->dA, c->dB, n, g_scr.vflag, g_fold_stream);
            }
            if (e == cudaSuccess) e = cudaEventCreateWithFlags(&c->validated, cudaEventDisableTiming);
            if (e == cudaSuccess) e = cudaEventRecord(c->validated, g_fold_stream);
            c->pending_validation = e == cudaSuccess;
        } else {
            Span sp(3, g_stream);
            launch_validate_points(c->dA, c->dB, n, g_scr.flag, g_stream);
        }
        g_stats.launches++;
    }
    int flag = 0;
    if (e == cudaSuccess) e = cudaMemcpyAsync(&flag, g_scr.flag, sizeof(int), cudaMemcpyDeviceToHost, g_stream);
    if (e == cudaSuccess) e = cudaStreamSynchronize(g_stream);
    if (e != cudaSuccess) { sipp_ctx_destroy(c); return cuda_fail(e, "decode"); }
    if (flag) {
        sipp_ctx_destroy(c);
        return fail(SIPP_ERR_ENCODING, (flag & 1) ? "input coordinate >= p" : (flag & 2) ? "input point is not on the curve"
                                                                                         : "input G2 point is not in the prime-order subgroup");
    }
    *out = c;
    return SIPP_OK;
}
int sipp_ctx_create_from_device(const void* dA, const void* dB, size_t n, sipp_ctx** out) { return ctx_create_from_device_ex(dA, dB, n, out, false); }

static int ctx_finish_validation(sipp_ctx* c) {
    if (!c || !c->pending_validation) return SIPP_OK;
    c->pending_validation = false;
    int flag = 0;
    cudaError_t e = cudaEventSynchronize(c->validated);
    if (e == cudaSuccess) e = cudaMemcpy(&flag, g_scr.vflag, sizeof(int), cudaMemcpyDeviceToHost);
    cudaEventDestroy(c->validated);
    c->validated = nullptr;
    if (e != cudaSuccess) return cuda_fail(e, "point validation");
    if (flag) return fail(SIPP_ERR_ENCODING, (flag & 2) ? "input point is not on the curve" : "input G2 point is not in the prime-order subgroup");
    return SIPP_OK;
}

static int ctx_create_ex(const uint8_t* A, const uint8_t* B, size_t n, sipp_ctx** out, bool defer);
static int ctx_create_ex(const uint8_t* A, const uint8_t* B, size_t n, sipp_ctx** out, bool defer) {
    int rc = ensure_init();
    if (rc) return rc;
    if (!A || !B || !out || n == 0) return fail(SIPP_ERR_ARG, "sipp_ctx_create: null pointer or n == 0");
    uint8_t *tA = nullptr, *tB = nullptr;
    CK(pool_alloc((void**)&tA, n * 64));
    cudaError_t e = pool_alloc((void**)&tB, n * 128);
    if (e != cudaSuccess) { pool_free(tA); return cuda_fail(e, "cudaMalloc"); }
    e = cudaMemcpyAsync(tA, A, n * 64, cudaMemcpyHostToDevice, g_stream);
    if (e == cudaSuccess) e = cudaMemcpyAsync(tB, B, n * 128, cudaMemcpyHostToDevice, g_stream);
    if (e != cudaSuccess) { pool_free(tA); pool_free(tB); return cuda_fail(e, "H2D"); }
    rc = ctx_create_from_device_ex(tA, tB, n, out, defer);
    pool_free(tA);
    pool_free(tB);
    return rc;
}

int sipp_ctx_create(const uint8_t* A, const uint8_t* B, size_t n, sipp_ctx** out) { return ctx_create_ex(A, B, n, out, false); }

int sipp_ctx_destroy(sipp_ctx* c) {
    if (!c) return SIPP_OK;
    if (c->pending_validation) {
        cudaEventSynchronize(c->validated);
        cudaEventDestroy(c->validated);
        c->pending_validation = false;
    }
    pool_free(c->dA);
    pool_free(c->dB);
    delete c;
    g_live_ctx--;
    return SIPP_OK;
}

size_t sipp_ctx_len(const sipp_ctx* c) { return c ? c->n : 0; }

int sipp_ctx_set_stages(sipp_ctx* c, int on) {
    if (!c) return fail(SIPP_ERR_ARG, "null ctx");
    if (c->mt.n) return fail(SIPP_ERR_ARG, "a pairing-matrix stage is in progress");
    c->stages = on != 0;
    return SIPP_OK;
}

int sipp_ctx_inner_product(sipp_ctx* c, uint8_t out[384]) {
    if (!c || !out) return fail(SIPP_ERR_ARG, "null argument");
    if (c->stages && !c->mt.n) {
        if (const size_t nr0 = mat_stage_first(c->n)) {
            int rc = mat_build(c, c->mt, nr0);
            return rc ? rc : mat_diag_product(c->mt, out);
        }
    }
    return ctx_products(c, 0, out, nullptr);
}

int sipp_ctx_cross_products(sipp_ctx* c, uint8_t zl[384], uint8_t zr[384]) {
    if (!c || !zl || !zr) return fail(SIPP_ERR_ARG, "null argument");
    if (c->stages) {
        if (c->n < 2) return fail(SIPP_ERR_ARG, "cross products need n >= 2");
        if (!c->mt.n) {
            const size_t nr = mat_stage(c->n);
            if (nr) {
                int rc = mat_build(c, c->mt, nr);
                if (rc) return rc;
            }
        }
        if (c->mt.n) return mat_products(c->mt, zl, zr);
    }
    return ctx_products(c, 1, zl, zr);
}

int sipp_ctx_fold(sipp_ctx* c, const uint8_t x[32], const uint8_t x_inv[32]) {
    if (!c || !x || !x_inv) return fail(SIPP_ERR_ARG, "null argument");
    if (c->n < 2) return fail(SIPP_ERR_ARG, "fold needs n >= 2");
    if (c->pending_validation) CK(cudaStreamWaitEvent(g_stream, c->validated, 0));
    if (c->mt.n) return mat_fold(c, c->mt, x, x_inv);
    size_t h = c->n / 2;
    FoldPlan plan;
    if (fold_plan_build(x, x_inv, &plan)) return fail(SIPP_ERR_ENCODING, "fold scalar out of range (must be < r)");
    {
        Span sp(2, g_stream);
        int e;
        if (g_opt_fold_straus && h >= 16384) {
            if (!g_fold_plan_dev) CK(cudaMalloc(&g_fold_plan_dev, sizeof(FoldPlan)));
            FoldPlan* d_plan = g_fold_plan_dev;
            CK(cudaMemcpyAsync(d_plan, &plan, sizeof plan, cudaMemcpyHostToDevice, g_stream));
            e = launch_fold_straus(c->dA, c->dB, h, c->n, 1, d_plan, g_stream);
        } else {
            e = h <= (size_t)g_opt_wide_fold_max ? launch_fold_wide(c->dA, c->dB, h, plan, g_stream) : launch_fold(c->dA, c->dB, h, plan, g_stream);
        }
        if (e) return cuda_fail((cudaError_t)e, "k_fold");
    }
    g_stats.launches += 1;
    g_stats.fold_points += h;
    c->n = h;
    return SIPP_OK;
}

int sipp_ctx_read(sipp_ctx* c, uint8_t* A_out, uint8_t* B_out) {
    if (!c) return fail(SIPP_ERR_ARG, "null ctx");
    if (c->stale) return fail(SIPP_ERR_ARG, "the points of this context were not folded during its pairing-matrix tail (sipp_ctx_set_stages)");
    if (c->mt.n && c->mt.fold_points) CK(order_after(g_stream, g_fold_stream));
    size_t n = c->n;
    uint32_t* tmp;
    CK(pool_alloc((void**)&tmp, n * 32 * sizeof(uint32_t)));
    cudaError_t e = cudaSuccess;
    if (A_out) {
        launch_codec_encode(c->dA, tmp, n * 2, g_stream);
        g_stats.launches++;
        e = cudaMemcpyAsync(A_out, tmp, n * 64, cudaMemcpyDeviceToHost, g_stream);
        if (e == cudaSuccess) e = cudaStreamSynchronize(g_stream);
    }
    if (B_out && e == cudaSuccess) {
        launch_codec_encode(c->dB, tmp, n * 4, g_stream);
        g_stats.launches++;
        e = cudaMemcpyAsync(B_out, tmp, n * 128, cudaMemcpyDeviceToHost, g_stream);
        if (e == cudaSuccess) e = cudaStreamSynchronize(g_stream);
    }
    pool_free(tmp);
    if (e != cudaSuccess) return cuda_fail(e, "sipp_ctx_read");
    return SIPP_OK;
}

int sipp_ctx_partial_products(sipp_ctx* c, int which, void* d_out, void* stream) {
    if (!c || !d_out) return fail(SIPP_ERR_ARG, "null argument");
    cudaStream_t s = stream ? (cudaStream_t)stream : cudaStreamLegacy;
    if (s != g_stream) CK(order_after(s, g_stream));
    size_t blocks;
    int nprod;
    int rc = ctx_products_to_device(c, which, &blocks, &nprod, s);
    if (rc) return rc;
    rc = launch_reduce(g_scr.partials, (int)blocks, nprod, (uint32_t*)d_out, false, s);
    if (rc) return rc;
    if (s != g_stream) CK(order_after(g_stream, s));
    return SIPP_OK;
}

int sipp_combine_partials(const void* d_partials, int count, int nprod, uint8_t* out, void* stream) {
    int rc = ensure_init();
    if (rc) return rc;
    if (!d_partials || !out || count < 1 || nprod < 1 || nprod > 2) return fail(SIPP_ERR_ARG, "bad argument");
    rc = scratch_reserve(1);
    if (rc) return rc;
    cudaStream_t s = stream ? (cudaStream_t)stream : cudaStreamLegacy;
    if (s != g_stream) CK(order_after(s, g_stream));
    rc = launch_reduce((const uint32_t*)d_partials, count, nprod, g_scr.out, true, s);
    if (rc) return rc;
    CK(cudaMemcpyAsync(g_scr.h_out, g_scr.out, (size_t)nprod * 384, cudaMemcpyDeviceToHost, s));
    CK(cudaStreamSynchronize(s));
    memcpy(out, g_scr.h_out, (size_t)nprod * 384);
    return SIPP_OK;
}

int sipp_inner_product(const uint8_t* A, const uint8_t* B, size_t n, uint8_t out[384]) {
    if (!out) return fail(SIPP_ERR_ARG, "null argument");
    if (n == 0) {
        memset(out, 0, 384);
        out[0] = 1;
        return ensure_init();
    }
    sipp_ctx* c;
    int rc = sipp_ctx_create(A, B, n, &c);
    if (rc) return rc;
    rc = sipp_ctx_inner_product(c, out);
    sipp_ctx_destroy(c);
    return rc;
}

int sipp_pairing(const uint8_t a[64], const uint8_t b[128], uint8_t out[384]) { return sipp_inner_product(a, b, 1, out); }

int sipp_gt_fold(const uint8_t zl[384], const uint8_t z[384], const uint8_t zr[384], const uint8_t x[32], const uint8_t x_inv[32],
                 uint8_t out[384]) {
    int rc = ensure_init();
    if (rc) return rc;
    if (!zl || !z || !zr || !x || !x_inv || !out) return fail(SIPP_ERR_ARG, "null argument");
    rc = scratch_reserve(1);
    if (rc) return rc;
    uint32_t* d_in;
    CK(cudaMalloc(&d_in, 3 * 384));
    cudaMemcpyAsync(d_in, zl, 384, cudaMemcpyHostToDevice, g_stream);
    cudaMemcpyAsync(d_in + 96, z, 384, cudaMemcpyHostToDevice, g_stream);
    cudaMemcpyAsync(d_in + 192, zr, 384, cudaMemcpyHostToDevice, g_stream);
    {
        Span sp(3, g_stream);
        if (g_opt_fe_engine) launch_gt_fold_eng(d_in, scalar_from_bytes(x), scalar_from_bytes(x_inv), g_scr.out, g_stream);
        else launch_gt_fold(d_in, scalar_from_bytes(x), scalar_from_bytes(x_inv), g_scr.out, g_stream);
    }
    g_stats.launches++;
    cudaError_t e = cudaMemcpyAsync(g_scr.h_out, g_scr.out, 384, cudaMemcpyDeviceToHost, g_stream);
    if (e == cudaSuccess) e = cudaStreamSynchronize(g_stream);
    cudaFree(d_in);
    if (e != cudaSuccess) return cuda_fail(e, "sipp_gt_fold");
    memcpy(out, g_scr.h_out, 384);
    return SIPP_OK;
}

int sipp_fr_inverse(const uint8_t x[32], uint8_t out[32]) {
    if (!x || !out) return fail(SIPP_ERR_ARG, "null argument");
    uint64_t v[4], r[4] = {0, 0, 0, 0};
    memcpy(v, x, 32);
    const int rc = sipp::glv::fr_inverse_binary(v, r);
    if (rc == -1) return fail(SIPP_ERR_ENCODING, "scalar >= r");
    if (rc == -2) return fail(SIPP_ERR_ZERO_CHALLENGE, "challenge is zero: x.inverse().unwrap() panics in the reference");
    memcpy(out, r, 32);
    return SIPP_OK;
}

size_t sipp_proof_len(size_t n) { return is_pow2(n) ? 2 * log2_exact(n) + 1 : 0; }

}
namespace sipp_host {
int prove_core(sipp_ctx* c, AbsorbJob& job, uint8_t* proof) {
    size_t n = c->n;
    size_t np = sipp_proof_len(n);
    std::vector<uint8_t> fwd(np * 384);
    size_t k = 0;
    sipp_transcript& tr = job.tr;
    c->stages = true;
    int rc = sipp_ctx_inner_product(c, &fwd[384 * k]);
    k++;
    bool first = true;
    while (rc == SIPP_OK && n > 1) {
        uint8_t* zl = &fwd[384 * k];
        uint8_t* zr = &fwd[384 * (k + 1)];
        rc = sipp_ctx_cross_products(c, zl, zr);
        if (rc) break;
        if (first) {
            g_stats.transcript_ms += job.join();
            sipp_transcript_append_fq12(&tr, &fwd[0]);
            first = false;
        }
        auto h0 = std::chrono::steady_clock::now();
        sipp_transcript_append_fq12(&tr, zl);
        sipp_transcript_append_fq12(&tr, zr);
        k += 2;
        uint8_t x[32], xinv[32];
        sipp_transcript_get_challenge(&tr, x);
        rc = sipp_fr_inverse(x, xinv);
        g_stats.transcript_ms += std::chrono::duration<double, std::milli>(std::chrono::steady_clock::now() - h0).count();
        if (rc) break;
        rc = sipp_ctx_fold(c, x, xinv);
        n = c->n;
    }
    if (rc) return rc;
    for (size_t i = 0; i < np; i++) memcpy(proof + 384 * i, &fwd[384 * (np - 1 - i)], 384);
    return SIPP_OK;
}
}
extern "C" {

int sipp_ctx_prove(sipp_ctx* c, const uint8_t* A, const uint8_t* B, uint8_t* proof) {
    if (!c || !A || !B || !proof) return fail(SIPP_ERR_ARG, "null argument");
    if (!is_pow2(c->n)) return fail(SIPP_ERR_ARG, "n must be a power of two (the reference halves n every round)");
    AbsorbJob job;
    job.start(A, B, c->n);
    return prove_core(c, job, proof);
}

int sipp_prove_native(const uint8_t* A, size_t a_len, const uint8_t* B, size_t b_len, uint8_t* proof) {
    if (a_len != b_len) return fail(SIPP_ERR_LENGTH, "assert_eq!(A.len(), B.len()) failed");
    if (!is_pow2(a_len)) return fail(SIPP_ERR_ARG, "n must be a non-zero power of two");
    if (!A || !B || !proof) return fail(SIPP_ERR_ARG, "null argument");
    int rc = ensure_init();
    if (rc) return rc;
    AbsorbJob job;
    job.start(A, B, a_len);
    sipp_ctx* c;
    rc = ctx_create_ex(A, B, a_len, &c, true);
    if (rc) return rc;
    rc = prove_core(c, job, proof);
    const int vrc = ctx_finish_validation(c);
    sipp_ctx_destroy(c);
    return vrc ? vrc : rc;
}

int sipp_verify_native(const uint8_t* A, size_t a_len, const uint8_t* B, size_t b_len, const uint8_t* proof, size_t proof_len, uint8_t* final_A,
                       uint8_t* final_B, uint8_t* final_Z) {
    if (!A || !B || !proof) return fail(SIPP_ERR_ARG, "null argument");
    if (a_len != b_len) return fail(SIPP_ERR_LENGTH, "A.len() != B.len()");
    size_t n = a_len;
    if (!is_pow2(n)) return fail(SIPP_ERR_ARG, "n must be a non-zero power of two");
    if (proof_len < sipp_proof_len(n)) return fail(SIPP_ERR_SHORT_PROOF, "proof.pop().unwrap() on an empty proof");
    if (!fq_bytes_canonical(proof + 384 * (proof_len - sipp_proof_len(n)), 12 * sipp_proof_len(n))) return fail(SIPP_ERR_ENCODING, "proof coordinate >= p");
    int rc = ensure_init();
    if (rc) return rc;
    AbsorbJob job;
    job.start(A, B, n);
    sipp_ctx* c;
    rc = ctx_create_ex(A, B, n, &c, true);
    if (rc) return rc;
    g_stats.transcript_ms += job.join();
    sipp_transcript& tr = job.tr;
    size_t top = proof_len;
    uint8_t Z[384];
    memcpy(Z, proof + 384 * --top, 384);
    sipp_transcript_append_fq12(&tr, Z);
    const size_t rounds = log2_exact(n);
    std::vector<uint8_t> xs(rounds * 64), elems((2 * rounds + 1) * 384);
    memcpy(elems.data(), Z, 384);
    for (size_t k = 0; k < rounds && !rc; k++) {
        const uint8_t* zl = proof + 384 * --top;
        sipp_transcript_append_fq12(&tr, zl);
        const uint8_t* zr = proof + 384 * --top;
        sipp_transcript_append_fq12(&tr, zr);
        sipp_transcript_get_challenge(&tr, &xs[64 * k]);
        rc = sipp_fr_inverse(&xs[64 * k], &xs[64 * k + 32]);
        memcpy(&elems[384 * (1 + 2 * k)], zl, 384);
        memcpy(&elems[384 * (2 + 2 * k)], zr, 384);
    }
    uint32_t *d_elems = nullptr, *d_xs = nullptr, *d_parts = nullptr, *d_z = nullptr;
    const bool gt_batched = !rc && rounds > 0 && g_opt_fe_engine;
    if (gt_batched) {
        if (!g_fold_stream) CK(cudaStreamCreateWithFlags(&g_fold_stream, cudaStreamNonBlocking));
        cudaError_t e = pool_alloc((void**)&d_elems, elems.size());
        if (e == cudaSuccess) e = pool_alloc((void**)&d_xs, xs.size());
        if (e == cudaSuccess) e = pool_alloc((void**)&d_parts, (rounds + 1) * 384);
        if (e == cudaSuccess) e = pool_alloc((void**)&d_z, 384);
        if (e == cudaSuccess) e = order_after(g_fold_stream, g_stream);
        if (e == cudaSuccess) e = cudaMemcpyAsync(d_elems, elems.data(), elems.size(), cudaMemcpyHostToDevice, g_fold_stream);
        if (e == cudaSuccess) e = cudaMemcpyAsync(d_xs, xs.data(), xs.size(), cudaMemcpyHostToDevice, g_fold_stream);
        int le = 0;
        if (e == cudaSuccess) {
            Span sp(3, g_fold_stream);
            le = launch_gt_fold_rounds(d_elems, d_xs, (int)rounds, d_parts, g_fold_stream);
            if (!le) le = launch_reduce_fe_eng(d_parts, (int)rounds + 1, 1, d_z, 2, g_opt_fe_norm, g_fold_stream);
            g_stats.launches += 2;
        }
        if (e == cudaSuccess && !le) e = cudaMemcpyAsync(Z, d_z, 384, cudaMemcpyDeviceToHost, g_fold_stream);
        if (e != cudaSuccess || le) {
            cudaStreamSynchronize(g_fold_stream);
            pool_free(d_elems); pool_free(d_xs); pool_free(d_parts); pool_free(d_z);
            sipp_ctx_destroy(c);
            return e != cudaSuccess ? cuda_fail(e, "verifier GT updates") : cuda_fail((cudaError_t)le, "k_gt_fold_rounds");
        }
    }
    for (size_t k = 0; k < rounds && !rc; k++) {
        rc = sipp_ctx_fold(c, &xs[64 * k], &xs[64 * k + 32]);
        if (!rc && !gt_batched) {
            uint8_t nz[384];
            rc = sipp_gt_fold(&elems[384 * (1 + 2 * k)], Z, &elems[384 * (2 + 2 * k)], &xs[64 * k], &xs[64 * k + 32], nz);
            if (!rc) memcpy(Z, nz, 384);
        }
    }
    n = c->n;
    if (gt_batched) {
        cudaError_t e = cudaStreamSynchronize(g_fold_stream);
        pool_free(d_elems); pool_free(d_xs); pool_free(d_parts); pool_free(d_z);
        if (e != cudaSuccess) { sipp_ctx_destroy(c); return cuda_fail(e, "verifier GT updates"); }
    }
    uint8_t fa[64], fb[128], e[384];
    if (!rc) rc = sipp_ctx_read(c, fa, fb);
    if (!rc) rc = sipp_ctx_inner_product(c, e);
    const int vrc = ctx_finish_validation(c);
    sipp_ctx_destroy(c);
    if (vrc) return vrc;
    if (rc) return rc;
    if (final_A) memcpy(final_A, fa, 64);
    if (final_B) memcpy(final_B, fb, 128);
    if (final_Z) memcpy(final_Z, Z, 384);
    if (memcmp(e, Z, 384) != 0) return fail(SIPP_ERR_VERIFY, "Verification failed");
    return SIPP_OK;
}

int sipp_test_fq_op(int op, const uint8_t* a, const uint8_t* b, uint8_t* out, size_t count) {
    int rc = ensure_init();
    if (rc) return rc;
    if (!a || !out || count == 0) return fail(SIPP_ERR_ARG, "bad argument");
    uint32_t *da, *db = nullptr, *dout;
    CK(cudaMalloc(&da, count * 32));
    CK(cudaMalloc(&dout, count * 32));
    if (b) { CK(cudaMalloc(&db, count * 32)); CK(cudaMemcpyAsync(db, b, count * 32, cudaMemcpyHostToDevice, g_stream)); }
    CK(cudaMemcpyAsync(da, a, count * 32, cudaMemcpyHostToDevice, g_stream));
    launch_test_fq_op(op, da, db, dout, count, g_stream);
    g_stats.launches++;
    cudaError_t e = cudaStreamSynchronize(g_stream);
    if (e == cudaSuccess) e = cudaMemcpyAsync(out, dout, count * 32, cudaMemcpyDeviceToHost, g_stream);
    if (e == cudaSuccess) e = cudaStreamSynchronize(g_stream);
    cudaFree(da); cudaFree(dout); if (db) cudaFree(db);
    if (e != cudaSuccess) return cuda_fail(e, "sipp_test_fq_op");
    return SIPP_OK;
}

int sipp_test_fq12_op(int op, const uint8_t* a, const uint8_t* b, uint8_t* out, size_t count) {
    int rc = ensure_init();
    if (rc) return rc;
    if (!a || !out || count == 0) return fail(SIPP_ERR_ARG, "bad argument");
    uint32_t *da, *db = nullptr, *dout;
    CK(cudaMalloc(&da, count * 384));
    CK(cudaMalloc(&dout, count * 384));
    if (b) { CK(cudaMalloc(&db, count * 384)); CK(cudaMemcpyAsync(db, b, count * 384, cudaMemcpyHostToDevice, g_stream)); }
    CK(cudaMemcpyAsync(da, a, count * 384, cudaMemcpyHostToDevice, g_stream));
    if (op >= 20) launch_test_coop_op(op - 20, da, db, dout, count, g_stream);
    else launch_test_fq12_op(op, da, db, dout, count, g_stream);
    g_stats.launches++;
    cudaError_t e = cudaStreamSynchronize(g_stream);
    if (e == cudaSuccess) e = cudaMemcpyAsync(out, dout, count * 384, cudaMemcpyDeviceToHost, g_stream);
    if (e == cudaSuccess) e = cudaStreamSynchronize(g_stream);
    cudaFree(da); cudaFree(dout); if (db) cudaFree(db);
    if (e != cudaSuccess) return cuda_fail(e, "sipp_test_fq12_op");
    return SIPP_OK;
}

int sipp_test_fold_plan(const uint8_t x[32], const uint8_t x_inv[32], uint32_t* out_words, size_t out_cap) {
    if (!x || !x_inv || !out_words || out_cap < sizeof(FoldPlan) / 4) return fail(SIPP_ERR_ARG, "bad argument");
    FoldPlan plan;
    if (fold_plan_build(x, x_inv, &plan)) return fail(SIPP_ERR_ENCODING, "fold scalar out of range (must be < r)");
    memcpy(out_words, &plan, sizeof plan);
    return (int)(sizeof(FoldPlan) / 4);
}

int sipp_microbench(int which, int iters, double* ops_per_s, double* ms_out) {
    int rc = ensure_init();
    if (rc) return rc;
    if (!ops_per_s || iters < 1) return fail(SIPP_ERR_ARG, "bad argument");
    const int threads = 256;
    const int blocks = g_sm_count * 8;
    uint64_t* d_out;
    CK(cudaMalloc(&d_out, (size_t)blocks * threads * sizeof(uint64_t)));
    cudaEvent_t a, b;
    CK(cudaEventCreate(&a));
    CK(cudaEventCreate(&b));
    double per_thread_ops = 0;
    float best = 1e30f;
    for (int rep = 0; rep < 4; rep++) {
        CK(cudaEventRecord(a, g_stream));
        if (launch_microbench(which, blocks, threads, d_out, iters, 12345u + rep, &per_thread_ops, g_stream)) {
            cudaFree(d_out);
            return fail(SIPP_ERR_ARG, "unknown microbenchmark or launch failure");
        }
        g_stats.launches++;
        CK(cudaEventRecord(b, g_stream));
        CK(cudaEventSynchronize(b));
        float ms;
        CK(cudaEventElapsedTime(&ms, a, b));
        if (rep > 0 && ms < best) best = ms;
    }
    cudaEventDestroy(a);
    cudaEventDestroy(b);
    cudaFree(d_out);
    *ops_per_s = per_thread_ops * threads * blocks / (best * 1e-3);
    if (ms_out) *ms_out = best;
    return SIPP_OK;
}

}
```

Baseline: 131,400.

## Group consecutive point folds into one multi-term fold launch

During the pairing-matrix tail, fold challenges are now buffered and up to g rounds of point folding are applied together. Each final point is computed as the sum of scalar multiples of 2^g-1 source points, using products of the pending challenges built on the host. Default group max is 2, and grouping only happens when the total term count fits the SM budget. This cuts the number of serial fold launches and intermediate affine conversions, at the cost of more scalar multiplications per output point and a scratch buffer.

```diff
diff --git a/include/sipp_b200.h b/include/sipp_b200.h
--- a/include/sipp_b200.h
+++ b/include/sipp_b200.h
@@ -43,6 +43,7 @@
 #define SIPP_OPT_MATRIX_BLOCK_N 15
 #define SIPP_OPT_MATRIX_FIRST 17
 #define SIPP_OPT_MATRIX_BLOCK_R 16
+#define SIPP_OPT_FOLD_GROUP_MAX 18
 int sipp_set_option(int option, int value);
 int sipp_get_option(int option);
 
@@ -157,6 +158,8 @@
 int sipp_test_fr_inverse_binary(const uint8_t x[32], uint8_t out[32]);
 int sipp_microbench(int which, int iters, double *ops_per_s, double *ms);
 long sipp_test_stage_blocks(int which, size_t n);
+int sipp_test_fold_groups(int rounds, size_t n, int *sizes_out, int cap);
+int sipp_test_fold_terms(const uint8_t *xs, int g, size_t n, uint32_t *offsets_out, uint32_t *plan_words, size_t plan_cap);
 long sipp_test_poseidon_chain(uint64_t seed, long count);
 int sipp_test_poseidon_scalar(int which, const uint64_t *in, uint64_t *out);
 const void *sipp_test_poseidon_tables(void);
diff --git a/sipp_b200/_lib.py b/sipp_b200/_lib.py
--- a/sipp_b200/_lib.py
+++ b/sipp_b200/_lib.py
@@ -7,6 +7,7 @@
 OK, ERR_CUDA, ERR_ARG, ERR_LENGTH, ERR_ZERO_CHALLENGE, ERR_SHORT_PROOF, ERR_ENCODING, ERR_VERIFY, ERR_COMM = 0, -1, -2, -3, -4, -5, -6, -7, -8
 OPT_FE_NORMALISATION, OPT_FQ12_ORDER, OPT_PROFILE, OPT_PIPELINE, OPT_WIDE_LINES_MAX, OPT_FE_ENGINE, OPT_WIDE_FOLD_MAX, OPT_WIDE_ACCUM_MAX = 1, 2, 3, 4, 5, 6, 7, 8
 OPT_BATCH_KPG_MAX, OPT_FOLD_STRAUS, OPT_BATCH_STREAMS, OPT_BATCH_QLINES, OPT_VALIDATE_POINTS, OPT_MATRIX_TAIL, OPT_MATRIX_BLOCK_N, OPT_MATRIX_BLOCK_R, OPT_MATRIX_FIRST = 9, 10, 11, 12, 13, 14, 15, 16, 17
+OPT_FOLD_GROUP_MAX = 18
 
 
 class SippError(RuntimeError):
diff --git a/sipp_b200/csrc/fold_plan.h b/sipp_b200/csrc/fold_plan.h
--- a/sipp_b200/csrc/fold_plan.h
+++ b/sipp_b200/csrc/fold_plan.h
@@ -25,9 +25,18 @@
     int bits;
 };
 
+#define SIPP_FOLD_GROUP_LIMIT 5
+#define SIPP_FOLD_TERMS_MAX ((1 << SIPP_FOLD_GROUP_LIMIT) - 1)
+struct FoldTerms {
+    FoldPlan plan[SIPP_FOLD_TERMS_MAX];
+    uint32_t off[SIPP_FOLD_TERMS_MAX];
+    int count;
+};
+
 int fold_decompose_g1(const uint64_t k[4], FoldSubScalar out[2]);
 int fold_decompose_g2(const uint64_t k[4], FoldSubScalar out[4]);
 int fold_plan_build(const uint8_t x[32], const uint8_t x_inv[32], FoldPlan* plan);
+int fold_terms_build(const uint8_t* xs, int g, size_t n, FoldTerms* terms);
 int gt_plan_build(const uint8_t x[32], const uint8_t x_inv[32], GtPlan* plan);
 
 }
diff --git a/sipp_b200/csrc/glv.cc b/sipp_b200/csrc/glv.cc
--- a/sipp_b200/csrc/glv.cc
+++ b/sipp_b200/csrc/glv.cc
@@ -21,6 +21,44 @@
     memcpy(ki, x_inv, 32);
     memset(plan, 0, sizeof *plan);
     return glv::plan_build(kx, ki, HOST_TABLES, plan);
+}
+
+static void fr_mul(const uint64_t a[4], const uint64_t b[4], uint64_t out[4]) {
+    static const uint64_t R2[4] = {0x1bb8e645ae216da7ull, 0x53fe3ab1e35c59e3ull, 0x8c49833d53bb8085ull, 0x0216d0b17f4e44a5ull};
+    uint64_t t[4];
+    glv::fr_mont_mul(t, a, b);
+    glv::fr_mont_mul(out, t, R2);
+}
+
+int fold_terms_build(const uint8_t* xs, int g, size_t n, FoldTerms* terms) {
+    if (g < 1 || g > SIPP_FOLD_GROUP_LIMIT || (n >> g) == 0 || (n >> 32)) return -1;
+    static const uint64_t M[4] = {0x43e1f593f0000001ull, 0x2833e84879b97091ull, 0xb85045b68181585dull, 0x30644e72e131a029ull};
+    uint64_t x[SIPP_FOLD_GROUP_LIMIT][2][4];
+    for (int j = 0; j < g; j++) {
+        memcpy(x[j][0], xs + 64 * j, 32);
+        memcpy(x[j][1], xs + 64 * j + 32, 32);
+        if (glv::fr_geq(x[j][0], M) || glv::fr_geq(x[j][1], M)) return -1;
+    }
+    memset(terms, 0, sizeof *terms);
+    terms->count = (1 << g) - 1;
+    uint64_t prod[SIPP_FOLD_TERMS_MAX + 1][2][4];
+    for (int S = 1; S <= terms->count; S++) {
+        const int j = __builtin_ctz(S), rest = S & (S - 1);
+        uint64_t off = (uint64_t)(n >> (j + 1));
+        if (rest) {
+            fr_mul(prod[rest][0], x[j][0], prod[S][0]);
+            fr_mul(prod[rest][1], x[j][1], prod[S][1]);
+            off += terms->off[rest - 1];
+        } else {
+            memcpy(prod[S], x[j], sizeof prod[S]);
+        }
+        terms->off[S - 1] = (uint32_t)off;
+        uint8_t kx[32], ki[32];
+        memcpy(kx, prod[S][0], 32);
+        memcpy(ki, prod[S][1], 32);
+        if (fold_plan_build(kx, ki, &terms->plan[S - 1])) return -1;
+    }
+    return 0;
 }
 
 int gt_plan_build(const uint8_t x[32], const uint8_t x_inv[32], GtPlan* plan) {
diff --git a/sipp_b200/csrc/host_state.h b/sipp_b200/csrc/host_state.h
--- a/sipp_b200/csrc/host_state.h
+++ b/sipp_b200/csrc/host_state.h
@@ -18,6 +18,8 @@
     size_t m = 1;
     bool fold_points = false;
     int folds = 0;
+    uint8_t pending[SIPP_FOLD_GROUP_LIMIT * 64];
+    int npending = 0, group = 1;
     void reset() {
         pool_free(E[0]);
         pool_free(E[1]);
@@ -25,6 +27,7 @@
         n = 0;
         m = 1;
         fold_points = false;
+        npending = 0;
     }
     ~MatTail() { reset(); }
 };
@@ -48,7 +51,7 @@
 extern cudaStream_t g_stream;
 #define SIPP_FIRST_STAGE_LOG2_LOOPS 18
 size_t mat_first_budget(size_t n);
-extern int g_opt_pipeline, g_opt_fe_norm, g_opt_fq12_order, g_opt_profile, g_opt_fold_straus, g_opt_batch_kpg_max, g_opt_batch_streams, g_opt_batch_qlines, g_opt_wide_max, g_opt_wide_fold_max, g_opt_fe_engine, g_opt_validate, g_opt_matrix_n, g_opt_matrix_first, g_opt_matrix_block_n, g_opt_matrix_block_r;
+extern int g_opt_pipeline, g_opt_fe_norm, g_opt_fq12_order, g_opt_profile, g_opt_fold_straus, g_opt_batch_kpg_max, g_opt_batch_streams, g_opt_batch_qlines, g_opt_wide_max, g_opt_wide_fold_max, g_opt_fe_engine, g_opt_validate, g_opt_matrix_n, g_opt_matrix_first, g_opt_matrix_block_n, g_opt_matrix_block_r, g_opt_fold_group_max;
 extern sipp_stats g_stats;
 
 int fail(int code, const char* what);
@@ -103,6 +106,7 @@
 int mat_adopt(MatTail& mt, const uint32_t* gathered, int ranks, size_t nr);
 int mat_products(MatTail& mt, uint8_t* zl, uint8_t* zr);
 int mat_fold(sipp_ctx* c, MatTail& mt, const uint8_t x[32], const uint8_t xinv[32]);
+int mat_flush_folds(sipp_ctx* c, MatTail& mt);
 
 int prove_core(sipp_ctx* c, AbsorbJob& job, uint8_t* proof);
 
diff --git a/sipp_b200/csrc/k_fold.cu b/sipp_b200/csrc/k_fold.cu
--- a/sipp_b200/csrc/k_fold.cu
+++ b/sipp_b200/csrc/k_fold.cu
@@ -164,6 +164,51 @@
     }
 }
 
+__global__ void __launch_bounds__(SIPP_FOLD_THREADS) k_fold_split_terms(const uint32_t* __restrict__ A, const uint32_t* __restrict__ B, size_t h,
+                                                                       FoldTerms terms, unsigned g2_blocks, uint32_t* __restrict__ scratch) {
+    __shared__ FoldPlan plan;
+    __shared__ __align__(16) uint32_t xch[3 * 32 * 48];
+    const int t = blockIdx.y;
+    for (int i = threadIdx.x; i < (int)(sizeof(FoldPlan) / 4); i += blockDim.x) ((uint32_t*)&plan)[i] = ((const uint32_t*)&terms.plan[t])[i];
+    __syncthreads();
+    const size_t off = terms.off[t];
+    const int warp = threadIdx.x >> 5, lane = threadIdx.x & 31;
+    if (blockIdx.x < g2_blocks) {
+        const int el = lane >> 1;
+        size_t i = (size_t)blockIdx.x * 16 + el;
+        const bool valid = i < h;
+        if (!valid) i = h - 1;
+        G2A q = endo_apply(load_g2(B, i + off), warp);
+        if (plan.g2[warp].neg) q.y = f_neg(q.y);
+        Jac<Fq2H> acc = jac_scalar_mul_naf(split_g2(q), plan.g2[warp].plus, plan.g2[warp].minus, plan.g2_bits);
+        if (warp > 0) store_jac_h(xch + ((warp - 1) * 16 + el) * 48, acc);
+        __syncthreads();
+        if (warp == 0) {
+#pragma unroll 1
+            for (int j = 0; j < 3; j++) acc = jac_add(acc, load_jac_h(xch + (j * 16 + el) * 48));
+            if (valid) store_jac_h(scratch + ((size_t)t * h + i) * 48, acc);
+        }
+    } else {
+        const int comp = warp & 1, half = warp >> 1, el = lane >> 1;
+        size_t i = (size_t)(blockIdx.x - g2_blocks) * 32 + half * 16 + el;
+        const bool valid = i < h;
+        if (!valid) i = h - 1;
+        G1A q = endo_apply(load_g1(A, i + off), comp);
+        if (plan.g1[comp].neg) q.y = fq_neg(q.y);
+        Jac<Fq> acc = jac_scalar_mul_naf_pair(q, plan.g1[comp].plus, plan.g1[comp].minus, plan.g1_bits);
+        if (comp == 1 && !h_odd()) store_jac(xch + (half * 16 + el) * 24, acc);
+        __syncthreads();
+        if (comp == 0 && !h_odd()) {
+            acc = jac_add(acc, load_jac1(xch + (half * 16 + el) * 24));
+            if (valid) store_jac(scratch + (size_t)terms.count * h * 48 + ((size_t)t * h + i) * 24, acc);
+        }
+    }
+}
+int launch_fold_split_terms(const uint32_t* A, const uint32_t* B, size_t h, const FoldTerms& terms, uint32_t* scratch, cudaStream_t s) {
+    const unsigned g2_blocks = (unsigned)((h + 15) / 16), g1_blocks = (unsigned)((h + 31) / 32);
+    k_fold_split_terms<<<dim3(g2_blocks + g1_blocks, (unsigned)terms.count), SIPP_FOLD_THREADS, 0, s>>>(A, B, h, terms, g2_blocks, scratch);
+    return (int)cudaGetLastError();
+}
 
 __global__ void __launch_bounds__(SIPP_FOLD_THREADS) k_fold_batch(uint32_t* __restrict__ A, uint32_t* __restrict__ B, size_t h, size_t stride, size_t count,
                                                                  const FoldPlan* __restrict__ plans, unsigned g2_blocks) {
diff --git a/sipp_b200/csrc/k_wide.cu b/sipp_b200/csrc/k_wide.cu
--- a/sipp_b200/csrc/k_wide.cu
+++ b/sipp_b200/csrc/k_wide.cu
@@ -122,6 +122,70 @@
     return v;
 }
 
+__device__ __forceinline__ void wide_g2_comp(DevMachine& mach, uint32_t* slots, uint32_t* o, const FoldPlan& plan, int comp, const uint32_t* B, size_t src) {
+    const FoldDigits d = fold_digits(plan.g2[comp], plan.g2_bits);
+    bool ident = false;
+    if (mach.lane == 0) {
+        G2A q = load_g2(B, src);
+        ident = affine_is_identity(q);
+        q = endo_apply(q, comp);
+        if ((plan.g2[comp].neg != 0) != d.flip) q.y = fq2_neg(q.y);
+        lp_fill_fixed(slots, fq_zero(), fq_zero(), q.x, q.y);
+    }
+    __syncwarp();
+    if (d.top >= 0) {
+        mach.run(SIPP_LP_SETUP_FIRST, SIPP_LP_SETUP_LEVELS);
+        lp_scalar_mul(mach, true, d.plus, d.minus, d.top);
+    }
+    if (mach.lane == 0) {
+        Jac<Fq2> r = jac_identity<Fq2>();
+        if (!ident && d.top >= 0) {
+            const Fq2 X{lp_load(slots, SIPP_LP_SLOT_X0), lp_load(slots, SIPP_LP_SLOT_X1)}, Y{lp_load(slots, SIPP_LP_SLOT_Y0), lp_load(slots, SIPP_LP_SLOT_Y1)};
+            const Fq2 Z = fq2_mul_xi(Fq2{lp_load(slots, SIPP_LP_SLOT_ZH0), lp_load(slots, SIPP_LP_SLOT_ZH1)});
+            r.x = fq2_mul(X, Z);
+            r.y = fq2_mul(Y, fq2_sqr(Z));
+            r.z = Z;
+        }
+        store_words(o, r.x.c0); store_words(o + 8, r.x.c1); store_words(o + 16, r.y.c0); store_words(o + 24, r.y.c1);
+        store_words(o + 32, r.z.c0); store_words(o + 40, r.z.c1);
+    }
+}
+__device__ __forceinline__ void wide_g1_comp(DevMachine& mach, uint32_t* slots, uint32_t* o, const FoldPlan& plan, int comp, const uint32_t* A, size_t src) {
+    const FoldDigits d = fold_digits(plan.g1[comp], plan.g1_bits);
+    bool ident = false;
+    if (mach.lane == 0) {
+        G1A q = load_g1(A, src);
+        ident = affine_is_identity(q);
+        q = endo_apply(q, comp);
+        if ((plan.g1[comp].neg != 0) != d.flip) q.y = fq_neg(q.y);
+        lp_store(slots, SIPP_LP_SLOT_ZERO, fq_zero());
+        lp_store(slots, SIPP_LP_SLOT_QX0, q.x); lp_store(slots, SIPP_LP_SLOT_QY0, q.y);
+        lp_store(slots, SIPP_LP_SLOT_X1, q.x); lp_store(slots, SIPP_LP_SLOT_Y1, q.y); lp_store(slots, SIPP_LP_SLOT_Z1, fq_one());
+    }
+    __syncwarp();
+    if (d.top >= 0) lp_scalar_mul(mach, false, d.plus, d.minus, d.top);
+    if (mach.lane == 0) {
+        Jac<Fq> r = jac_identity<Fq>();
+        if (!ident && d.top >= 0) {
+            const Fq X = lp_load(slots, SIPP_LP_SLOT_X1), Y = lp_load(slots, SIPP_LP_SLOT_Y1), Z = lp_load(slots, SIPP_LP_SLOT_Z1);
+            r.x = fq_mul(X, Z);
+            r.y = fq_mul(Y, fq_sqr(Z));
+            r.z = Z;
+        }
+        store_words(o, r.x); store_words(o + 8, r.y); store_words(o + 16, r.z);
+    }
+}
+__device__ __forceinline__ Jac<Fq2> load_jac2(const uint32_t* o) {
+    Jac<Fq2> t;
+    t.x = Fq2{load_words(o), load_words(o + 8)}; t.y = Fq2{load_words(o + 16), load_words(o + 24)}; t.z = Fq2{load_words(o + 32), load_words(o + 40)};
+    return t;
+}
+__device__ __forceinline__ Jac<Fq> load_jac1(const uint32_t* o) {
+    Jac<Fq> t;
+    t.x = load_words(o); t.y = load_words(o + 8); t.z = load_words(o + 16);
+    return t;
+}
+
 __global__ void __launch_bounds__(SIPP_WIDE_THREADS) k_fold_wide(uint32_t* __restrict__ A, uint32_t* __restrict__ B, size_t h, FoldPlan plan_arg, unsigned g2_blocks) {
     __shared__ __align__(16) uint32_t smem[SIPP_WIDE_GROUPS * SIPP_LP_SLOTS * 8];
     __shared__ FoldPlan plan;
@@ -137,40 +201,12 @@
         size_t e = (size_t)blockIdx.x * 2 + gi;
         const bool valid = e < h;
         if (!valid) e = h - 1;
-        const FoldDigits d = fold_digits(plan.g2[comp], plan.g2_bits);
-        bool ident = false;
-        if (lane == 0) {
-            G2A q = load_g2(B, e + h);
-            ident = affine_is_identity(q);
-            q = endo_apply(q, comp);
-            if ((plan.g2[comp].neg != 0) != d.flip) q.y = fq2_neg(q.y);
-            lp_fill_fixed(slots, fq_zero(), fq_zero(), q.x, q.y);
-        }
-        __syncwarp();
-        if (d.top >= 0) {
-            mach.run(SIPP_LP_SETUP_FIRST, SIPP_LP_SETUP_LEVELS);
-            lp_scalar_mul(mach, true, d.plus, d.minus, d.top);
-        }
-        if (lane == 0) {
-            Jac<Fq2> r = jac_identity<Fq2>();
-            if (!ident && d.top >= 0) {
-                const Fq2 X{lp_load(slots, SIPP_LP_SLOT_X0), lp_load(slots, SIPP_LP_SLOT_X1)}, Y{lp_load(slots, SIPP_LP_SLOT_Y0), lp_load(slots, SIPP_LP_SLOT_Y1)};
-                const Fq2 Z = fq2_mul_xi(Fq2{lp_load(slots, SIPP_LP_SLOT_ZH0), lp_load(slots, SIPP_LP_SLOT_ZH1)});
-                r.x = fq2_mul(X, Z);
-                r.y = fq2_mul(Y, fq2_sqr(Z));
-                r.z = Z;
-            }
-            uint32_t* o = xch + group * 48;
-            store_words(o, r.x.c0); store_words(o + 8, r.x.c1); store_words(o + 16, r.y.c0); store_words(o + 24, r.y.c1);
-            store_words(o + 32, r.z.c0); store_words(o + 40, r.z.c1);
-        }
+        wide_g2_comp(mach, slots, xch + group * 48, plan, comp, B, e + h);
         __syncthreads();
         if (warp == 0 && lane == 0) {
             Jac<Fq2> acc;
             for (int j = 0; j < 4; j++) {
-                const uint32_t* o = xch + ((j * 2 + gi) * 48);
-                Jac<Fq2> t;
-                t.x = Fq2{load_words(o), load_words(o + 8)}; t.y = Fq2{load_words(o + 16), load_words(o + 24)}; t.z = Fq2{load_words(o + 32), load_words(o + 40)};
+                const Jac<Fq2> t = load_jac2(xch + ((j * 2 + gi) * 48));
                 acc = j ? jac_add(acc, t) : t;
             }
             const G2A r = jac_to_affine(jac_add_affine(acc, load_g2(B, e)));
@@ -181,41 +217,69 @@
         size_t e = (size_t)(blockIdx.x - g2_blocks) * 4 + pair * 2 + gi;
         const bool valid = e < h;
         if (!valid) e = h - 1;
-        const FoldDigits d = fold_digits(plan.g1[comp], plan.g1_bits);
-        bool ident = false;
-        if (lane == 0) {
-            G1A q = load_g1(A, e + h);
-            ident = affine_is_identity(q);
-            q = endo_apply(q, comp);
-            if ((plan.g1[comp].neg != 0) != d.flip) q.y = fq_neg(q.y);
-            lp_store(slots, SIPP_LP_SLOT_ZERO, fq_zero());
-            lp_store(slots, SIPP_LP_SLOT_QX0, q.x); lp_store(slots, SIPP_LP_SLOT_QY0, q.y);
-            lp_store(slots, SIPP_LP_SLOT_X1, q.x); lp_store(slots, SIPP_LP_SLOT_Y1, q.y); lp_store(slots, SIPP_LP_SLOT_Z1, fq_one());
-        }
-        __syncwarp();
-        if (d.top >= 0) lp_scalar_mul(mach, false, d.plus, d.minus, d.top);
-        if (lane == 0) {
-            Jac<Fq> r = jac_identity<Fq>();
-            if (!ident && d.top >= 0) {
-                const Fq X = lp_load(slots, SIPP_LP_SLOT_X1), Y = lp_load(slots, SIPP_LP_SLOT_Y1), Z = lp_load(slots, SIPP_LP_SLOT_Z1);
-                r.x = fq_mul(X, Z);
-                r.y = fq_mul(Y, fq_sqr(Z));
-                r.z = Z;
-            }
-            uint32_t* o = xch + group * 48;
-            store_words(o, r.x); store_words(o + 8, r.y); store_words(o + 16, r.z);
-        }
+        wide_g1_comp(mach, slots, xch + group * 48, plan, comp, A, e + h);
         __syncthreads();
         if (comp == 0 && lane == 0) {
-            Jac<Fq> acc, t;
-            const uint32_t* o0 = xch + group * 48;
-            const uint32_t* o1 = xch + (group + 2) * 48;
-            acc.x = load_words(o0); acc.y = load_words(o0 + 8); acc.z = load_words(o0 + 16);
-            t.x = load_words(o1); t.y = load_words(o1 + 8); t.z = load_words(o1 + 16);
-            acc = jac_add(acc, t);
+            const Jac<Fq> acc = jac_add(load_jac1(xch + group * 48), load_jac1(xch + (group + 2) * 48));
             const G1A r = jac_to_affine(jac_add_affine(acc, load_g1(A, e)));
             if (valid) store_g1(A, e, r);
         }
+    }
+}
+
+__global__ void __launch_bounds__(SIPP_WIDE_THREADS) k_fold_terms(const uint32_t* __restrict__ A, const uint32_t* __restrict__ B, size_t h, FoldTerms terms,
+                                                                  unsigned g2_blocks, uint32_t* __restrict__ scratch) {
+    __shared__ __align__(16) uint32_t smem[SIPP_WIDE_GROUPS * SIPP_LP_SLOTS * 8];
+    __shared__ FoldPlan plan;
+    __shared__ __align__(16) uint32_t xch[SIPP_WIDE_GROUPS * 48];
+    const int t = blockIdx.y;
+    for (int i = threadIdx.x; i < (int)(sizeof(FoldPlan) / 4); i += blockDim.x) ((uint32_t*)&plan)[i] = ((const uint32_t*)&terms.plan[t])[i];
+    __syncthreads();
+    const size_t off = terms.off[t];
+    const int warp = threadIdx.x >> 5, group = threadIdx.x / SIPP_LP_LANES, lane = threadIdx.x % SIPP_LP_LANES, gi = group & 1;
+    uint32_t* slots = smem + group * (SIPP_LP_SLOTS * 8);
+    DevMachine mach;
+    mach.slots = slots; mach.out = nullptr; mach.lane = lane; mach.store = false; mach.ident = false;
+    if (blockIdx.x < g2_blocks) {
+        size_t e = (size_t)blockIdx.x * 2 + gi;
+        const bool valid = e < h;
+        if (!valid) e = h - 1;
+        wide_g2_comp(mach, slots, xch + group * 48, plan, warp, B, e + off);
+        __syncthreads();
+        if (warp == 0 && lane == 0 && valid) {
+            Jac<Fq2> acc = load_jac2(xch + gi * 48);
+            for (int j = 1; j < 4; j++) acc = jac_add(acc, load_jac2(xch + ((j * 2 + gi) * 48)));
+            uint32_t* o = scratch + ((size_t)t * h + e) * 48;
+            store_words(o, acc.x.c0); store_words(o + 8, acc.x.c1); store_words(o + 16, acc.y.c0); store_words(o + 24, acc.y.c1);
+            store_words(o + 32, acc.z.c0); store_words(o + 40, acc.z.c1);
+        }
+    } else {
+        const int comp = warp & 1, pair = warp >> 1;
+        size_t e = (size_t)(blockIdx.x - g2_blocks) * 4 + pair * 2 + gi;
+        const bool valid = e < h;
+        if (!valid) e = h - 1;
+        wide_g1_comp(mach, slots, xch + group * 48, plan, comp, A, e + off);
+        __syncthreads();
+        if (comp == 0 && lane == 0 && valid) {
+            const Jac<Fq> acc = jac_add(load_jac1(xch + group * 48), load_jac1(xch + (group + 2) * 48));
+            uint32_t* o = scratch + (size_t)terms.count * h * 48 + ((size_t)t * h + e) * 24;
+            store_words(o, acc.x); store_words(o + 8, acc.y); store_words(o + 16, acc.z);
+        }
+    }
+}
+
+__global__ void __launch_bounds__(64) k_fold_terms_sum(uint32_t* __restrict__ A, uint32_t* __restrict__ B, size_t h, int count, const uint32_t* __restrict__ scratch) {
+    const size_t th = (size_t)blockIdx.x * blockDim.x + threadIdx.x;
+    if (th < h) {
+        Jac<Fq2> acc = load_jac2(scratch + th * 48);
+        for (int t = 1; t < count; t++) acc = jac_add(acc, load_jac2(scratch + ((size_t)t * h + th) * 48));
+        store_g2(B, th, jac_to_affine(jac_add_affine(acc, load_g2(B, th))));
+    } else if (th < 2 * h) {
+        const size_t e = th - h;
+        const uint32_t* s1 = scratch + (size_t)count * h * 48;
+        Jac<Fq> acc = load_jac1(s1 + e * 24);
+        for (int t = 1; t < count; t++) acc = jac_add(acc, load_jac1(s1 + ((size_t)t * h + e) * 24));
+        store_g1(A, e, jac_to_affine(jac_add_affine(acc, load_g1(A, e))));
     }
 }
 
@@ -332,5 +396,19 @@
     k_fold_wide<<<g2_blocks + g1_blocks, SIPP_WIDE_THREADS, 0, s>>>(A, B, h, plan, g2_blocks);
     return (int)cudaGetLastError();
 }
-
-}
+size_t fold_terms_scratch_bytes(size_t h, int count) { return (size_t)count * h * (48 + 24) * sizeof(uint32_t); }
+int launch_fold_terms(uint32_t* A, uint32_t* B, size_t h, const FoldTerms& terms, bool split, uint32_t* scratch, cudaStream_t s) {
+    const unsigned g2_blocks = (unsigned)((h + 1) / 2), g1_blocks = (unsigned)((h + 3) / 4);
+    if (split) {
+        const int e = launch_fold_split_terms(A, B, h, terms, scratch, s);
+        if (e) return e;
+    } else {
+        k_fold_terms<<<dim3(g2_blocks + g1_blocks, (unsigned)terms.count), SIPP_WIDE_THREADS, 0, s>>>(A, B, h, terms, g2_blocks, scratch);
+    }
+    cudaError_t e = cudaGetLastError();
+    if (e != cudaSuccess) return (int)e;
+    k_fold_terms_sum<<<(unsigned)((2 * h + 63) / 64), 64, 0, s>>>(A, B, h, terms.count, scratch);
+    return (int)cudaGetLastError();
+}
+
+}
diff --git a/sipp_b200/csrc/launch.h b/sipp_b200/csrc/launch.h
--- a/sipp_b200/csrc/launch.h
+++ b/sipp_b200/csrc/launch.h
@@ -34,6 +34,9 @@
 int launch_gt_fold_rounds(const uint32_t* elems, const uint32_t* scalars, int rounds, uint32_t* partials, cudaStream_t s);
 int launch_fold(uint32_t* A, uint32_t* B, size_t h, const FoldPlan& plan, cudaStream_t s);
 int launch_fold_wide(uint32_t* A, uint32_t* B, size_t h, const FoldPlan& plan, cudaStream_t s);
+size_t fold_terms_scratch_bytes(size_t h, int count);
+int launch_fold_terms(uint32_t* A, uint32_t* B, size_t h, const FoldTerms& terms, bool split, uint32_t* scratch, cudaStream_t s);
+int launch_fold_split_terms(const uint32_t* A, const uint32_t* B, size_t h, const FoldTerms& terms, uint32_t* scratch, cudaStream_t s);
 int launch_validate_points(const uint32_t* dA, const uint32_t* dB, size_t n, int* flags, cudaStream_t s);
 int launch_test_fq_op(int op, const uint32_t* a, const uint32_t* b, uint32_t* out, size_t count, cudaStream_t s);
 int launch_test_fq12_op(int op, const uint32_t* a, const uint32_t* b, uint32_t* out, size_t count, cudaStream_t s);
diff --git a/sipp_b200/csrc/sipp_b200.cu b/sipp_b200/csrc/sipp_b200.cu
--- a/sipp_b200/csrc/sipp_b200.cu
+++ b/sipp_b200/csrc/sipp_b200.cu
@@ -31,6 +31,7 @@
 int g_opt_matrix_first = 1;
 int g_opt_matrix_block_n = 256, g_opt_matrix_block_r = 8;
 int g_opt_validate = 1;
+int g_opt_fold_group_max = 2;
 
 struct TimedSpan {
     cudaEvent_t a, b;
@@ -304,6 +305,8 @@
 namespace sipp_host {
 cudaStream_t g_fold_stream = nullptr;
 FoldPlan* g_fold_plan_dev = nullptr;
+uint32_t* g_fold_terms_scratch = nullptr;
+size_t g_fold_terms_bytes = 0;
 int g_live_ctx = 0;
 
 size_t mat_stage(size_t n) {
@@ -462,7 +465,49 @@
     return SIPP_OK;
 }
 
+size_t fold_terms_fit_wide() { return (size_t)g_sm_count * 8 / 3; }
+int mat_fold_group(size_t rounds, size_t n) {
+    const int g = (int)((rounds - 1) % (size_t)g_opt_fold_group_max) + 1;
+    const size_t element_terms = (n >> g) * (((size_t)1 << g) - 1), fits = (size_t)g_sm_count * 128 / 3;
+    return g > 1 && element_terms > fits ? 1 : g;
+}
+
+int mat_flush_folds(sipp_ctx* c, MatTail& mt) {
+    const int g = mt.npending;
+    if (!g) return SIPP_OK;
+    mt.npending = 0;
+    const size_t h = c->n;
+    int le;
+    if (g == 1) {
+        FoldPlan fp;
+        if (fold_plan_build(mt.pending, mt.pending + 32, &fp)) return fail(SIPP_ERR_ENCODING, "fold scalar out of range (must be < r)");
+        Span sp(2, g_fold_stream);
+        le = h <= (size_t)g_opt_wide_fold_max ? launch_fold_wide(c->dA, c->dB, h, fp, g_fold_stream) : launch_fold(c->dA, c->dB, h, fp, g_fold_stream);
+    } else {
+        FoldTerms terms;
+        if (fold_terms_build(mt.pending, g, h << g, &terms)) return fail(SIPP_ERR_ENCODING, "fold scalar out of range (must be < r)");
+        const size_t bytes = fold_terms_scratch_bytes(h, terms.count);
+        if (bytes > g_fold_terms_bytes) {
+            if (g_fold_terms_scratch) CK(cudaFree(g_fold_terms_scratch));
+            g_fold_terms_scratch = nullptr;
+            g_fold_terms_bytes = 0;
+            CK(cudaMalloc(&g_fold_terms_scratch, bytes));
+            g_fold_terms_bytes = bytes;
+        }
+        Span sp(2, g_fold_stream);
+        le = launch_fold_terms(c->dA, c->dB, h, terms, h * (size_t)terms.count > fold_terms_fit_wide(), g_fold_terms_scratch, g_fold_stream);
+        g_stats.launches++;
+    }
+    if (le) return cuda_fail((cudaError_t)le, "k_fold (look-ahead stage)");
+    g_stats.launches++;
+    return SIPP_OK;
+}
+
 int mat_fold(sipp_ctx* c, MatTail& mt, const uint8_t x[32], const uint8_t xinv[32]) {
+    if (mt.fold_points && mt.folds++ == 0) {
+        if (!g_fold_stream) CK(cudaStreamCreateWithFlags(&g_fold_stream, cudaStreamNonBlocking));
+        CK(order_after(g_fold_stream, g_stream));
+    }
     if (mt.n > 2) {
         GtPlan plan;
         if (gt_plan_build(x, xinv, &plan)) return fail(SIPP_ERR_ENCODING, "fold scalar out of range (must be < r)");
@@ -474,19 +519,19 @@
     }
     const size_t h = c->n / 2;
     if (mt.fold_points) {
-        FoldPlan fp;
-        if (fold_plan_build(x, xinv, &fp)) return fail(SIPP_ERR_ENCODING, "fold scalar out of range (must be < r)");
-        if (!g_fold_stream) CK(cudaStreamCreateWithFlags(&g_fold_stream, cudaStreamNonBlocking));
-        if (mt.folds++ == 0) CK(order_after(g_fold_stream, g_stream));
-        Span sp(2, g_fold_stream);
-        int le = h <= (size_t)g_opt_wide_fold_max ? launch_fold_wide(c->dA, c->dB, h, fp, g_fold_stream) : launch_fold(c->dA, c->dB, h, fp, g_fold_stream);
-        if (le) return cuda_fail((cudaError_t)le, "k_fold (look-ahead stage)");
-        g_stats.launches++;
+        if (mt.npending == 0) mt.group = mat_fold_group(log2_exact(mt.n), c->n);
+        memcpy(mt.pending + 64 * mt.npending, x, 32);
+        memcpy(mt.pending + 64 * mt.npending + 32, xinv, 32);
+        mt.npending++;
     }
     if (!mt.fold_points) c->stale = true;
     g_stats.fold_points += h;
     c->n = h;
     mt.n /= 2;
+    if (mt.fold_points && (mt.npending == mt.group || mt.n == 1)) {
+        int rc = mat_flush_folds(c, mt);
+        if (rc) return rc;
+    }
     if (mt.n == 1) {
         if (mt.fold_points) CK(order_after(g_stream, g_fold_stream));
         mt.reset();
@@ -554,6 +599,9 @@
     batch_release_streams();
     if (g_fold_plan_dev) cudaFree(g_fold_plan_dev);
     g_fold_plan_dev = nullptr;
+    if (g_fold_terms_scratch) cudaFree(g_fold_terms_scratch);
+    g_fold_terms_scratch = nullptr;
+    g_fold_terms_bytes = 0;
     if (g_stream) cudaStreamDestroy(g_stream);
     g_stream = nullptr;
     if (g_fold_stream) cudaStreamDestroy(g_fold_stream);
@@ -587,10 +635,35 @@
             if (value < 4 || value > 32 || (value & (value - 1))) return fail(SIPP_ERR_ARG, "SIPP_OPT_MATRIX_BLOCK_R: 4, 8, 16 or 32");
             g_opt_matrix_block_r = value;
             return SIPP_OK;
+        case SIPP_OPT_FOLD_GROUP_MAX:
+            if (value < 1 || value > SIPP_FOLD_GROUP_LIMIT) return fail(SIPP_ERR_ARG, "SIPP_OPT_FOLD_GROUP_MAX: 1 to 5");
+            g_opt_fold_group_max = value;
+            return SIPP_OK;
         default: return fail(SIPP_ERR_ARG, "unknown option");
     }
 }
 long sipp_test_stage_blocks(int which, size_t n) { return (long)(which == 0 ? mat_stage_first(n) : mat_stage(n)); }
+int sipp_test_fold_groups(int rounds, size_t n, int* sizes_out, int cap) {
+    if (rounds < 1 || !sizes_out || (n >> rounds) == 0) return fail(SIPP_ERR_ARG, "bad argument");
+    int count = 0;
+    for (int r = rounds; r > 0;) {
+        const int g = mat_fold_group((size_t)r, n);
+        if (count == cap) return fail(SIPP_ERR_ARG, "sizes_out too small");
+        sizes_out[count++] = g;
+        r -= g;
+        n >>= g;
+    }
+    return count;
+}
+int sipp_test_fold_terms(const uint8_t* xs, int g, size_t n, uint32_t* offsets_out, uint32_t* plan_words, size_t plan_cap) {
+    if (!xs || !offsets_out || !plan_words) return fail(SIPP_ERR_ARG, "null argument");
+    FoldTerms terms;
+    if (fold_terms_build(xs, g, n, &terms)) return fail(SIPP_ERR_ARG, "bad group size, n or scalar");
+    if (plan_cap < (size_t)terms.count * (sizeof(FoldPlan) / 4)) return fail(SIPP_ERR_ARG, "plan_words too small");
+    memcpy(offsets_out, terms.off, terms.count * sizeof(uint32_t));
+    memcpy(plan_words, terms.plan, terms.count * sizeof(FoldPlan));
+    return terms.count;
+}
 int sipp_get_option(int option) {
     switch (option) {
         case SIPP_OPT_FE_NORMALISATION: return g_opt_fe_norm;
@@ -610,6 +683,7 @@
         case SIPP_OPT_MATRIX_FIRST: return g_opt_matrix_first;
         case SIPP_OPT_MATRIX_BLOCK_N: return g_opt_matrix_block_n;
         case SIPP_OPT_MATRIX_BLOCK_R: return g_opt_matrix_block_r;
+        case SIPP_OPT_FOLD_GROUP_MAX: return g_opt_fold_group_max;
         default: return -1;
     }
 }
@@ -784,7 +858,11 @@
 int sipp_ctx_read(sipp_ctx* c, uint8_t* A_out, uint8_t* B_out) {
     if (!c) return fail(SIPP_ERR_ARG, "null ctx");
     if (c->stale) return fail(SIPP_ERR_ARG, "the points of this context were not folded during its pairing-matrix tail (sipp_ctx_set_stages)");
-    if (c->mt.n && c->mt.fold_points) CK(order_after(g_stream, g_fold_stream));
+    if (c->mt.n && c->mt.fold_points) {
+        int rc = mat_flush_folds(c, c->mt);
+        if (rc) return rc;
+        CK(order_after(g_stream, g_fold_stream));
+    }
     size_t n = c->n;
     uint32_t* tmp;
     CK(pool_alloc((void**)&tmp, n * 32 * sizeof(uint32_t)));
```

Result: faster. 136,000, median of 6 (+3.5%).
